# rchiaramo/wavefront_path_tracer

Hardware: AMD Instinct MI355X
Metric: Mrays/s (extend+shade) at 1920×1080, 64 spp, 8 bounces; 1/2/4/8 GPU (higher is better)
Workload: dtype f32

## Files before the change

include/wfpt.h:

```cpp
#ifndef WFPT_H
#define WFPT_H

#include <stddef.h>
#include <stdint.h>

#ifdef __cplusplus
extern "C" {
#endif


typedef struct wfpt_sphere {
    float center[4];
    float radius;
    uint32_t material_idx;
    uint32_t material_type;
    uint32_t _buffer;
} wfpt_sphere;

typedef struct wfpt_material {
    float albedo[4];
    float fuzz;
    float refract_index;
    uint32_t material_type;
    uint32_t _buffer;
// ... 69 lines not shown
                       offsetof(wfpt_ray, pixel_idx) == 44,
                   "Ray: extend.wgsl:17-22, 48 bytes");
WFPT_LAYOUT_ASSERT(sizeof(wfpt_hit_payload) == 16 && offsetof(wfpt_hit_payload, ray_idx) == 4 && offsetof(wfpt_hit_payload, sphere_idx) == 8 &&
                       offsetof(wfpt_hit_payload, mat_type) == 12,
                   "HitPayload: extend.wgsl:24-29, 16 bytes");


typedef enum wfpt_status {
    WFPT_OK = 0,
    WFPT_ERR_INVALID_ARGUMENT = -1,
    WFPT_ERR_HIP = -2,
    WFPT_ERR_OUT_OF_MEMORY = -3,
    WFPT_ERR_UNSUPPORTED = -4,
    WFPT_ERR_NO_DEVICE = -5
} wfpt_status;

typedef enum wfpt_stage {
    WFPT_STAGE_GENERATE_RAYS = 0,
    WFPT_STAGE_EXTEND = 1,
    WFPT_STAGE_SHADE = 2,
    WFPT_STAGE_MISS = 3,
    WFPT_STAGE_ACCUMULATE = 4,
    WFPT_STAGE_SHADE_LAMBERTIAN = 5,
    WFPT_STAGE_SHADE_METAL = 6,
    WFPT_STAGE_SHADE_DIELECTRIC = 7,
    WFPT_STAGE_SCAN = 8,
    WFPT_STAGE_BOUNCE_FIRST = 9,
    WFPT_STAGE_BOUNCE = 10,
    WFPT_STAGE_BOUNCE_LAST = 11,
    WFPT_STAGE_COMPACT = 12,
    WFPT_STAGE_COUNT = 13
} wfpt_stage;

typedef enum wfpt_rng_mode { WFPT_RNG_DISPATCH = 0, WFPT_RNG_PIXEL = 1 } wfpt_rng_mode;

enum {
    WFPT_FLAG_SPLIT_SHADE = 1u << 0,
    WFPT_FLAG_NO_GRAPH = 1u << 1,
    WFPT_FLAG_UNFUSED = 1u << 2,
    WFPT_FLAG_BINARY_BVH = 1u << 3,
    WFPT_FLAG_NO_REFILL = 1u << 4,
    WFPT_FLAG_NO_LDS_SCENE = 1u << 5,
    WFPT_FLAG_EXACT_TRAVERSAL = 1u << 6,
    WFPT_FLAG_NO_BINNING = 1u << 7,
    WFPT_FLAG_BINNING = 1u << 8,
    WFPT_FLAG_AOV = 1u << 10,
    WFPT_FLAG_DENOISE = 1u << 11,
    WFPT_FLAG_ENVIRONMENT = 1u << 12 ,
    WFPT_FLAG_TEXTURES = 1u << 13    ,
    WFPT_FLAG_EMISSION = 1u << 14    ,
    WFPT_FLAG_NEE = 1u << 15         ,
    WFPT_FLAG_ENV_NEE = 1u << 16     ,
    WFPT_FLAG_MIS = 1u << 17         ,
    WFPT_FLAG_ENV_MIS = 1u << 18
};

#define WFPT_INACTIVE_PIXEL 0xffffffffu

typedef struct wfpt_params {
    uint32_t width;
    uint32_t height;
    uint32_t max_pixels;
    uint32_t max_wavefronts;
    uint32_t miss_floor;
    uint32_t rng_mode;
    uint32_t flags;
    uint32_t tile_rank;
    uint32_t tile_world;
    int32_t device;
    uint32_t batch;
} wfpt_params;

typedef struct wfpt_ctx wfpt_ctx;


uint32_t wfpt_scene_new(wfpt_sphere *spheres, wfpt_material *materials);
uint32_t wfpt_scene_book_one_final(uint64_t seed, wfpt_sphere *spheres, wfpt_material *materials, uint32_t capacity);
int wfpt_build_bvh(wfpt_sphere *spheres, uint32_t n_spheres, wfpt_bvh_node *nodes, uint32_t node_capacity,
                   uint32_t *n_nodes);
int wfpt_build_bvh_triangles(wfpt_triangle *triangles, uint32_t n_triangles, wfpt_bvh_node *nodes,
                             uint32_t node_capacity, uint32_t *n_nodes, uint32_t n_bins);
int wfpt_build_bvh_device(wfpt_sphere *spheres, uint32_t n_spheres, wfpt_bvh_node *nodes, uint32_t node_capacity,
                          uint32_t *n_nodes, int device, float *device_ms);
int wfpt_build_bvh_triangles_device(wfpt_triangle *triangles, uint32_t n_triangles, wfpt_bvh_node *nodes,
                                    uint32_t node_capacity, uint32_t *n_nodes, uint32_t n_bins, int device,
                                    float *device_ms);
int wfpt_load_obj(const char *path, wfpt_triangle *triangles, uint32_t capacity, uint32_t *n_triangles,
                  uint32_t material_idx, uint32_t material_type);
int wfpt_load_obj_uv(const char *path, wfpt_triangle *triangles, float *uv6, uint32_t capacity, uint32_t *n_triangles,
                     uint32_t material_idx, uint32_t material_type);
uint32_t wfpt_scene_random_mesh(uint64_t seed, uint32_t n_triangles, wfpt_triangle *triangles, wfpt_material *materials);
void wfpt_camera_new(const float look_from[3], const float look_at[3], float *pitch, float *yaw);
void wfpt_view_transform(const float position[3], float pitch, float yaw, float view[16]);
void wfpt_p_inv(float vfov_rad, float aspect_ratio, float z_near, float z_far, float p_inv[16]);
void wfpt_gpu_camera_new(const float position[3], float pitch, float yaw, float defocus_angle_rad,
                         float focus_distance, wfpt_gpu_camera *out);
float wfpt_to_radians(float degrees);
void wfpt_camera_controller_update(float position[3], float *pitch, float *yaw, const float amounts[6],
                                   float rotate[2], float speed, float sensitivity, float dt);
void wfpt_workgroup_size_64(uint32_t x, uint32_t *gx, uint32_t *gy);
int wfpt_stage_from_name(const char *name);
const char *wfpt_stage_name(int stage);


int wfpt_device_count(void);
wfpt_ctx *wfpt_create(const wfpt_params *params,
                      const wfpt_sphere *spheres, uint32_t n_spheres,
// ... 146 lines not shown
int wfpt_emission_timing_ms(wfpt_ctx *ctx, float *ms_total, uint32_t *launches);

int wfpt_nee_light_count(wfpt_ctx *ctx);
int wfpt_nee_timing_ms(wfpt_ctx *ctx, float *ms_total, uint32_t *launches);
int wfpt_sample_lights(wfpt_ctx *ctx, const float *in9, size_t n, float *out8);

int wfpt_set_environment_share(wfpt_ctx *ctx, float share);
float wfpt_environment_share(const wfpt_ctx *ctx);
int wfpt_read_environment_distribution(wfpt_ctx *ctx, uint32_t *row_wh, uint64_t *marg_h);
int wfpt_sample_environment_light(wfpt_ctx *ctx, const float *in10, size_t n, float *out8);

int wfpt_sample_lights_mis(wfpt_ctx *ctx, const float *in9, size_t n, float *out12);
int wfpt_mis_hit_weight(wfpt_ctx *ctx, const float *in8, size_t n, float *out4);

int wfpt_sample_environment_light_mis(wfpt_ctx *ctx, const float *in10, size_t n, float *out12);
int wfpt_env_mis_miss_weight(wfpt_ctx *ctx, const float *dirs3, size_t n, float *out4);


uint32_t wfpt_n_pixels(const wfpt_ctx *ctx);
uint32_t wfpt_ray_capacity(const wfpt_ctx *ctx);
int wfpt_read_accumulated(wfpt_ctx *ctx, float *rgb, size_t n_floats);
int wfpt_read_image(wfpt_ctx *ctx, float *rgb, size_t n_floats);
int wfpt_copy_accumulated_to_device(wfpt_ctx *ctx, void *device_ptr, size_t n_bytes);
#define WFPT_COMM_UNIQUE_ID_BYTES 128
int wfpt_comm_unique_id(void *id128);
int wfpt_comm_init(wfpt_ctx *ctx, const void *id128, int rank, int world);
int wfpt_gather_accumulated(wfpt_ctx *ctx);
int wfpt_gather_accumulated_timed(wfpt_ctx *ctx, float *ms);
int wfpt_read_gathered(wfpt_ctx *ctx, float *rgb, size_t n_floats);
int wfpt_comm_destroy(wfpt_ctx *ctx);

int wfpt_read_rays(wfpt_ctx *ctx, wfpt_ray *rays, uint32_t n);
int wfpt_read_extension_rays(wfpt_ctx *ctx, wfpt_ray *rays, uint32_t n);
int wfpt_read_hits(wfpt_ctx *ctx, wfpt_hit_payload *hits, uint32_t n);
int wfpt_read_misses(wfpt_ctx *ctx, uint32_t *ray_indices, uint32_t n);
int wfpt_write_rays(wfpt_ctx *ctx, const wfpt_ray *rays, uint32_t n);
int wfpt_read_bounce_table(wfpt_ctx *ctx, uint32_t *rows4, uint32_t max_rows, uint32_t *n_rows);
int wfpt_read_totals(wfpt_ctx *ctx, uint64_t totals[3]);
int wfpt_read_wavefront_totals(wfpt_ctx *ctx, uint64_t *rows3, uint32_t max_rows, uint32_t *n_rows);
int wfpt_device_info(int device, uint32_t *compute_units, uint32_t *memory_clock_khz, uint32_t *memory_bus_width_bits,
                     uint64_t *total_memory_bytes);
void wfpt_tonemap_rgb8(const float *accumulated, uint32_t n_pixels, uint32_t n_samples, uint8_t *rgb);

int wfpt_save_ppm(wfpt_ctx *ctx, const char *path);
int wfpt_save_pfm(wfpt_ctx *ctx, const char *path);
int wfpt_save_png(wfpt_ctx *ctx, const char *path);
int wfpt_write_png_rgb8(const char *path, const uint8_t *rgb, uint32_t width, uint32_t height);

int wfpt_selftest_math(int device, int op, const float *a, const float *b, float *out, size_t n);
int wfpt_debug_extend_blocks_per_cu(int device, uint32_t lds_bytes);
int wfpt_debug_read_stamps(wfpt_ctx *ctx, uint64_t out[16], int reset);
int wfpt_debug_read_stamps_ex(wfpt_ctx *ctx, int which, uint64_t out[16], int reset);
int wfpt_debug_bvh4(const wfpt_bvh_node *nodes, uint32_t n_nodes, uint32_t counts[4]);
const char *wfpt_build_info(void);

#ifdef __cplusplus
}
#endif
#endif
```

wavefront_path_tracer_amd/__init__.py:

```python
import ctypes as C
import os

import numpy as np

from . import _build

__all__ = ["SPP", "SPF", "Scene", "BVHTree", "Camera", "CameraController", "ProjectionMatrix", "GPUFrameBuffer",
           "RenderParameters", "RenderProgress", "Kernel", "PathTracer", "WfptError", "workgroup_size_64",
           "RNG_DISPATCH", "RNG_PIXEL", "FLAG_SPLIT_SHADE", "FLAG_NO_GRAPH", "FLAG_UNFUSED", "FLAG_BINARY_BVH", "FLAG_NO_REFILL", "FLAG_NO_LDS_SCENE", "FLAG_EXACT_TRAVERSAL", "FLAG_NO_BINNING", "FLAG_BINNING", "FLAG_AOV", "AOVS", "FLAG_DENOISE", "DENOISE_DEFAULTS", "FLAG_ENVIRONMENT", "load_environment", "FLAG_TEXTURES", "MAX_TEXTURES", "load_texture", "FLAG_EMISSION", "FLAG_NEE", "FLAG_ENV_NEE", "FLAG_MIS", "FLAG_ENV_MIS", "TEMPORAL_DEFAULTS", "TEMPORAL_OUTPUTS", "STAGES", "lib", "build",
           "tonemap_rgb8", "selftest_math", "device_count"]

SPP = 10
SPF = 1

RNG_DISPATCH, RNG_PIXEL = 0, 1
LOOP_KINDS = ("stages", "fused", "fused_binned", "refill")
FLAG_SPLIT_SHADE, FLAG_NO_GRAPH, FLAG_UNFUSED, FLAG_BINARY_BVH, FLAG_NO_REFILL, FLAG_NO_LDS_SCENE, FLAG_EXACT_TRAVERSAL, FLAG_NO_BINNING, FLAG_BINNING = 1, 2, 4, 8, 16, 32, 64, 128, 256
FLAG_AOV = 1 << 10
FLAG_ENVIRONMENT = 1 << 12
FLAG_TEXTURES = 1 << 13
MAX_TEXTURES = 64
TEXTURE_FILTERS = {"bilinear": 0, "nearest": 1}
FLAG_EMISSION = 1 << 14
FLAG_NEE = 1 << 15
FLAG_ENV_NEE = 1 << 16
FLAG_MIS = 1 << 17
FLAG_ENV_MIS = 1 << 18
FLAG_DENOISE = 1 << 11
DENOISE_DEFAULTS = {"iterations": 5, "sigma_luminance": 4.0, "sigma_normal": 128.0, "sigma_depth": 1.0, "sigma_albedo": 0.5}
TEMPORAL_DEFAULTS = {**DENOISE_DEFAULTS, "history_cap": 32.0, "depth_tolerance": 0.05, "normal_cos": 0.9}
TEMPORAL_OUTPUTS = {"color": (0, 3), "moments": (1, 2), "length": (2, 1), "motion": (3, 3)}
INACTIVE_PIXEL = 0xFFFFFFFF
AOV_ALBEDO, AOV_NORMAL, AOV_DEPTH, AOV_COVERAGE, AOV_PRIM_ID, AOV_MATERIAL_ID = 0, 1, 2, 3, 4, 5
AOVS = {"albedo": (AOV_ALBEDO, 3, "<f4"), "normal": (AOV_NORMAL, 3, "<f4"), "depth": (AOV_DEPTH, 1, "<f4"),
        "coverage": (AOV_COVERAGE, 1, "<f4"), "prim_id": (AOV_PRIM_ID, 1, "<u4"), "material_id": (AOV_MATERIAL_ID, 1, "<u4")}
STAGES = {"generate_rays": 0, "extend": 1, "shade": 2, "miss_kernel": 3, "accumulate": 4,
          "shade_lambertian": 5, "shade_metal": 6, "shade_dielectric": 7, "scan": 8,
          "bounce_first": 9, "bounce": 10, "bounce_last": 11, "compact": 12}
STAGE_COUNT = 13

SPHERE = np.dtype([("center", "<f4", 4), ("radius", "<f4"), ("material_idx", "<u4"),
                   ("material_type", "<u4"), ("_buffer", "<u4")])
MATERIAL = np.dtype([("albedo", "<f4", 4), ("fuzz", "<f4"), ("refract_index", "<f4"),
                     ("material_type", "<u4"), ("_buffer", "<u4")])
BVH_NODE = np.dtype([("aabb_min", "<f4", 3), ("left_first", "<u4"), ("aabb_max", "<f4", 3),
                     ("prim_count", "<u4")])
GPU_CAMERA = np.dtype([("position", "<f4", 4), ("pitch", "<f4"), ("yaw", "<f4"),
                       ("defocus_radius", "<f4"), ("focus_distance", "<f4")])
RAY = np.dtype([("origin", "<f4", 4), ("direction", "<f4", 4), ("inv_direction", "<f4", 3),
                ("pixel_idx", "<u4")])
HIT = np.dtype([("t", "<f4"), ("ray_idx", "<u4"), ("sphere_idx", "<u4"), ("mat_type", "<u4")])
TRIANGLE = np.dtype([("v0", "<f4", 3), ("material_idx", "<u4"), ("e1", "<f4", 3), ("material_type", "<u4"),
                     ("e2", "<f4", 3), ("_pad", "<u4")])


OK, ERR_INVALID_ARGUMENT, ERR_HIP, ERR_OUT_OF_MEMORY, ERR_UNSUPPORTED, ERR_NO_DEVICE = 0, -1, -2, -3, -4, -5


class WfptError(RuntimeError):
    def __init__(self, status, message):
        super().__init__(f"wfpt status {status}: {message}")
        self.status = status


class _Params(C.Structure):
    _fields_ = [("width", C.c_uint32), ("height", C.c_uint32), ("max_pixels", C.c_uint32),
                ("max_wavefronts", C.c_uint32), ("miss_floor", C.c_uint32), ("rng_mode", C.c_uint32),
                ("flags", C.c_uint32), ("tile_rank", C.c_uint32), ("tile_world", C.c_uint32),
                ("device", C.c_int32), ("batch", C.c_uint32)]


class _DenoiseParams(C.Structure):
    _fields_ = [("iterations", C.c_uint32), ("sigma_luminance", C.c_float), ("sigma_normal", C.c_float), ("sigma_depth", C.c_float),
                ("sigma_albedo", C.c_float), ("_reserved", C.c_uint32 * 3)]


class _EnvironmentParams(C.Structure):
    _fields_ = [("intensity", C.c_float), ("rotation", C.c_float), ("_reserved", C.c_uint32 * 6)]


# ... 188 lines not shown
        "wfpt_build_info": (C.c_char_p, []),
        "wfpt_save_ppm": (i32, [vp, C.c_char_p]),
        "wfpt_save_pfm": (i32, [vp, C.c_char_p]),
        "wfpt_save_png": (i32, [vp, C.c_char_p]),
        "wfpt_write_png_rgb8": (i32, [C.c_char_p, vp, u32, u32]),
        "wfpt_debug_extend_blocks_per_cu": (i32, [i32, u32]),
        "wfpt_debug_read_stamps": (i32, [vp, vp, i32]),
        "wfpt_debug_read_stamps_ex": (i32, [vp, i32, vp, i32]),
        "wfpt_debug_bvh4": (i32, [vp, u32, vp]),
        "wfpt_aov_channels": (i32, [i32]),
        "wfpt_read_aov": (i32, [vp, i32, vp, sz]),
        "wfpt_copy_aov_to_device": (i32, [vp, i32, vp, sz]),
        "wfpt_aov_timing_ms": (i32, [vp, C.POINTER(f32), C.POINTER(u32)]),
        "wfpt_denoise_params_default": (None, [C.POINTER(_DenoiseParams)]),
        "wfpt_denoise": (i32, [vp, C.POINTER(_DenoiseParams), vp, sz]),
        "wfpt_denoise_to_device": (i32, [vp, C.POINTER(_DenoiseParams), vp, sz]),
        "wfpt_read_variance": (i32, [vp, vp, sz]),
        "wfpt_denoise_timing_ms": (i32, [vp, C.POINTER(f32), C.POINTER(u32)]),
        "wfpt_set_frame_offset": (i32, [vp, u32]),
        "wfpt_frame_offset": (u32, [vp]),
        "wfpt_temporal_params_default": (None, [C.POINTER(_TemporalParams)]),
        "wfpt_denoise_temporal": (i32, [vp, C.POINTER(_TemporalParams), vp, sz]),
        "wfpt_denoise_temporal_to_device": (i32, [vp, C.POINTER(_TemporalParams), vp, sz]),
        "wfpt_read_temporal": (i32, [vp, i32, vp, sz]),
        "wfpt_reset_history": (i32, [vp]),
        "wfpt_temporal_timing_ms": (i32, [vp, C.POINTER(f32), C.POINTER(u32)]),
        "wfpt_environment_params_default": (None, [C.POINTER(_EnvironmentParams)]),
        "wfpt_set_environment": (i32, [vp, vp, u32, u32, C.POINTER(_EnvironmentParams)]),
        "wfpt_clear_environment": (i32, [vp]),
        "wfpt_sample_environment": (i32, [vp, vp, sz, vp]),
        "wfpt_texture_params_default": (None, [C.POINTER(_TextureParams)]),
        "wfpt_set_texture": (i32, [vp, u32, vp, u32, u32, C.POINTER(_TextureParams)]),
        "wfpt_clear_texture": (i32, [vp, u32]),
        "wfpt_bind_texture": (i32, [vp, u32, C.c_int32]),
        "wfpt_set_triangle_uvs": (i32, [vp, vp, u32]),
        "wfpt_sample_texture": (i32, [vp, u32, vp, sz, vp]),
        "wfpt_texture_timing_ms": (i32, [vp, C.POINTER(f32), C.POINTER(u32)]),
        "wfpt_load_obj_uv": (i32, [C.c_char_p, vp, vp, u32, C.POINTER(u32), u32, u32]),
        "wfpt_set_emission": (i32, [vp, u32, C.POINTER(f32)]),
        "wfpt_get_emission": (i32, [vp, u32, C.POINTER(f32)]),
        "wfpt_clear_emission": (i32, [vp]),
        "wfpt_emission_timing_ms": (i32, [vp, C.POINTER(f32), C.POINTER(u32)]),
        "wfpt_nee_light_count": (i32, [vp]),
        "wfpt_nee_timing_ms": (i32, [vp, C.POINTER(f32), C.POINTER(u32)]),
        "wfpt_sample_lights": (i32, [vp, vp, sz, vp]),
        "wfpt_set_environment_share": (i32, [vp, f32]),
        "wfpt_environment_share": (f32, [vp]),
        "wfpt_read_environment_distribution": (i32, [vp, vp, vp]),
        "wfpt_sample_environment_light": (i32, [vp, vp, sz, vp]),
        "wfpt_sample_lights_mis": (i32, [vp, vp, sz, vp]),
        "wfpt_mis_hit_weight": (i32, [vp, vp, sz, vp]),
        "wfpt_sample_environment_light_mis": (i32, [vp, vp, sz, vp]),
        "wfpt_env_mis_miss_weight": (i32, [vp, vp, sz, vp]),
    }
    for name, (res, args) in sig.items():
        fn = getattr(L, name)
        fn.restype = res
        fn.argtypes = args
    _lib = L
    return L


ABI_SYMBOLS = None


def abi_symbols():
    import re
    hdr = os.path.join(_build.ROOT, "include", "wfpt.h")
    text = open(hdr).read()
    text = re.sub(r"/\*.*?\*/", "", text, flags=re.S)
    return sorted(set(re.findall(r"\b(wfpt_[a-z0-9_]+)\s*\(", text)))


def _p(a):
    return a.ctypes.data_as(C.c_void_p)


def device_count():
    return lib().wfpt_device_count()


def comm_unique_id():
    buf = np.zeros(128, np.uint8)
    st = lib().wfpt_comm_unique_id(_p(buf))
    if st != 0:
        raise WfptError(st, lib().wfpt_last_error(None).decode())
    return buf.tobytes()


def device_info(device=0):
    cu, clk, width, mem = C.c_uint32(), C.c_uint32(), C.c_uint32(), C.c_uint64()
    st = lib().wfpt_device_info(device, C.byref(cu), C.byref(clk), C.byref(width), C.byref(mem))
    if st != 0:
        raise WfptError(st, lib().wfpt_last_error(None).decode())
    return {"compute_units": cu.value, "memory_clock_khz": clk.value, "memory_bus_width_bits": width.value,
            "total_memory_bytes": mem.value}


def workgroup_size_64(x):
    gx, gy = C.c_uint32(), C.c_uint32()
    lib().wfpt_workgroup_size_64(x, C.byref(gx), C.byref(gy))
    return gx.value, gy.value


def tonemap_rgb8(accumulated, n_samples):
    a = np.ascontiguousarray(accumulated, "<f4").reshape(-1)
    out = np.zeros(a.size, np.uint8)
    lib().wfpt_tonemap_rgb8(_p(a), a.size // 3, n_samples, _p(out))
    return out.reshape(-1, 3)


def write_png(path, rgb8, width, height):
    a = np.ascontiguousarray(rgb8, np.uint8)
    if a.size != 3 * width * height:
        raise ValueError("rgb8 must hold width * height RGB pixels")
    st = lib().wfpt_write_png_rgb8(os.fsencode(path), _p(a), width, height)
    if st != 0:
        raise WfptError(st, f"cannot write {path}")


def load_environment(path):
    data = open(path, "rb").read()
    if data[:2] in (b"PF", b"Pf"):
        return _read_pfm(data)
    if data[:2] == b"#?":
        return _read_hdr(data)
    raise ValueError(f"load_environment: {path} is neither a Radiance .hdr nor a .pfm file")

# ... 665 lines not shown
        n = int(np.prod(shape))
        want = ("float32",) if dtype == "<f4" else ("int32", "uint32")
        dt = str(getattr(tensor, "dtype", "")).replace("torch.", "")
        if dt not in want:
            raise TypeError(f"aov_to_tensor({name!r}): tensor dtype {dt or type(tensor).__name__} is not {' or '.join(want)}")
        if tensor.numel() != n:
            raise ValueError(f"aov_to_tensor({name!r}): tensor has {tensor.numel()} elements, the AOV {n} {shape}")
        if not tensor.is_contiguous():
            raise ValueError(f"aov_to_tensor({name!r}): tensor is not contiguous")
        if getattr(tensor, "device", None) is None or tensor.device.type != "cuda" or tensor.device.index != self._params.device:
            raise ValueError(f"aov_to_tensor({name!r}): tensor must live on this context's device (cuda:{self._params.device})")
        self._check(lib().wfpt_copy_aov_to_device(self.handle, which, C.c_void_p(tensor.data_ptr()), 4 * n))
        return tensor

    def aov_timing(self):
        ms, n = C.c_float(0.0), C.c_uint32(0)
        self._check(lib().wfpt_aov_timing_ms(self.handle, C.byref(ms), C.byref(n)))
        return float(ms.value), int(n.value)

    def variance(self):
        a = np.zeros((self.n_pixels // self.width, self.width), "<f4")
        self._check(lib().wfpt_read_variance(self.handle, _p(a), a.size))
        return a

    @staticmethod
    def _denoise_params(params):
        unknown = set(params) - set(DENOISE_DEFAULTS)
        if unknown:
            raise TypeError(f"unknown denoise parameter(s) {sorted(unknown)}: one of {sorted(DENOISE_DEFAULTS)}")
        v = {**DENOISE_DEFAULTS, **params}
        return _DenoiseParams(int(v["iterations"]), v["sigma_luminance"], v["sigma_normal"], v["sigma_depth"], v["sigma_albedo"])

    def denoise(self, **params):
        p = self._denoise_params(params)
        a = np.zeros((self.n_pixels // self.width, self.width, 3), "<f4")
        self._check(lib().wfpt_denoise(self.handle, C.byref(p), _p(a), a.size))
        return a

    def denoise_to_tensor(self, tensor, **params):
        p = self._denoise_params(params)
        n = self.n_pixels * 3
        dt = str(getattr(tensor, "dtype", "")).replace("torch.", "")
        if dt != "float32":
            raise TypeError(f"denoise_to_tensor: tensor dtype {dt or type(tensor).__name__} is not float32")
        if tensor.numel() != n:
            raise ValueError(f"denoise_to_tensor: tensor has {tensor.numel()} elements, the image {n}")
        if not tensor.is_contiguous():
            raise ValueError("denoise_to_tensor: tensor is not contiguous")
        if getattr(tensor, "device", None) is None or tensor.device.type != "cuda" or tensor.device.index != self._params.device:
            raise ValueError(f"denoise_to_tensor: tensor must live on this context's device (cuda:{self._params.device})")
        self._check(lib().wfpt_denoise_to_device(self.handle, C.byref(p), C.c_void_p(tensor.data_ptr()), 4 * n))
        return tensor

    def denoise_timing(self):
        ms, n = C.c_float(0.0), C.c_uint32(0)
        self._check(lib().wfpt_denoise_timing_ms(self.handle, C.byref(ms), C.byref(n)))
        return float(ms.value), int(n.value)

    def set_frame_offset(self, offset):
        self._check(lib().wfpt_set_frame_offset(self.handle, int(offset) & 0xFFFFFFFF))

    @property
    def frame_offset(self):
        return int(lib().wfpt_frame_offset(self.handle))

    @staticmethod
    def _temporal_params(params):
        unknown = set(params) - set(TEMPORAL_DEFAULTS)
        if unknown:
            raise TypeError(f"unknown temporal denoise parameter(s) {sorted(unknown)}: one of {sorted(TEMPORAL_DEFAULTS)}")
        v = {**TEMPORAL_DEFAULTS, **params}
        spatial = PathTracer._denoise_params({k: v[k] for k in DENOISE_DEFAULTS})
        return _TemporalParams(spatial, v["history_cap"], v["depth_tolerance"], v["normal_cos"])

    def denoise_temporal(self, **params):
        p = self._temporal_params(params)
        a = np.zeros((self.n_pixels // self.width, self.width, 3), "<f4")
        self._check(lib().wfpt_denoise_temporal(self.handle, C.byref(p), _p(a), a.size))
        return a

    def denoise_temporal_to_tensor(self, tensor, **params):
        p = self._temporal_params(params)
        n = self.n_pixels * 3
        dt = str(getattr(tensor, "dtype", "")).replace("torch.", "")
        if dt != "float32":
            raise TypeError(f"denoise_temporal_to_tensor: tensor dtype {dt or type(tensor).__name__} is not float32")
        if tensor.numel() != n:
            raise ValueError(f"denoise_temporal_to_tensor: tensor has {tensor.numel()} elements, the image {n}")
        if not tensor.is_contiguous():
            raise ValueError("denoise_temporal_to_tensor: tensor is not contiguous")
        if getattr(tensor, "device", None) is None or tensor.device.type != "cuda" or tensor.device.index != self._params.device:
            raise ValueError(f"denoise_temporal_to_tensor: tensor must live on this context's device (cuda:{self._params.device})")
        self._check(lib().wfpt_denoise_temporal_to_device(self.handle, C.byref(p), C.c_void_p(tensor.data_ptr()), 4 * n))
        return tensor

    def temporal(self, name):
        if name not in TEMPORAL_OUTPUTS:
            raise KeyError(f"unknown temporal output {name!r}: one of {sorted(TEMPORAL_OUTPUTS)}")
        which, ch = TEMPORAL_OUTPUTS[name]
        h = self.n_pixels // self.width
        a = np.zeros((h, self.width, ch) if ch > 1 else (h, self.width), "<f4")
        self._check(lib().wfpt_read_temporal(self.handle, which, _p(a), a.size))
        return a

    def reset_history(self):
        self._check(lib().wfpt_reset_history(self.handle))
# ... 270 lines not shown
```

wavefront_path_tracer_amd/_build.py:

```python
import os
import shutil
import subprocess

PKG_DIR = os.path.dirname(os.path.abspath(__file__))
ROOT = os.path.dirname(PKG_DIR)
CSRC = os.path.join(PKG_DIR, "csrc")
LIB_PATH = os.path.join(PKG_DIR, "libwfpt.so")
SOURCES = ["wfpt_kernels.hip", "wfpt_api.hip", "wfpt_bvh_build.hip", "wfpt_host.cpp"]
HEADERS = [os.path.join(CSRC, "wfpt_kernels.h"), os.path.join(CSRC, "wfpt_bvh4.h"), os.path.join(CSRC, "wfpt_device_math.h"),
           os.path.join(ROOT, "include", "wfpt.h")]
FLAGS = ["--offload-arch=gfx950", "-O3", "-std=c++17", "-fPIC", "-shared", "-ffp-contract=off",
         "-fhip-fp32-correctly-rounded-divide-sqrt", "-fno-fast-math", "-Wall", "-Wno-unused-function"]


def hipcc():
    exe = shutil.which("hipcc") or "/opt/rocm/bin/hipcc"
    if not os.path.exists(exe):
        raise RuntimeError("hipcc not found: libwfpt.so cannot be built (and there is no CPU fallback)")
    return exe


def stale():
    if not os.path.exists(LIB_PATH):
        return True
    t = os.path.getmtime(LIB_PATH)
    deps = [os.path.join(CSRC, s) for s in SOURCES] + HEADERS + [os.path.abspath(__file__)]
    return any(os.path.getmtime(d) > t for d in deps)


BUILD_INFO = os.path.join(PKG_DIR, "build_info.json")


def source_digest():
    import hashlib
    h = hashlib.sha256()
    for f in [os.path.join(CSRC, s) for s in SOURCES] + HEADERS:
        h.update(os.path.basename(f).encode() + b"\0")
        h.update(open(f, "rb").read())
    return h.hexdigest()


def write_build_info():
    import datetime
    import json

    def git(*a):
        try:
            return subprocess.run(["git", "-C", ROOT] + list(a), stdout=subprocess.PIPE, stderr=subprocess.DEVNULL, text=True, timeout=20).stdout.strip()
        except Exception:
            return ""
    info = {"git_head": git("rev-parse", "HEAD") or None, "git_dirty": bool(git("status", "--porcelain", "--untracked-files=no")),
            "built_utc": datetime.datetime.utcnow().strftime("%Y-%m-%dT%H:%M:%SZ"), "source_sha256": source_digest(),
            "flags": FLAGS + os.environ.get("WFPT_EXTRA_FLAGS", "").split()}
    try:
        json.dump(info, open(BUILD_INFO, "w"), indent=1)
    except OSError:
        pass
    return info


def build_info():
    import json
# ... 33 lines not shown
```

wavefront_path_tracer_amd/csrc/wfpt_api.hip:

```cpp
#include "wfpt_kernels.h"

#include <dlfcn.h>
#include <rccl/rccl.h>

#include <algorithm>
#include <cfloat>
#include <cmath>
#include <cstdio>
#include <cstdlib>
#include <cstring>
#include <deque>
#include <map>
#include <memory>
#include <string>
#include <type_traits>
#include <vector>

using namespace wfpt;

namespace {
thread_local std::string g_last_error;
thread_local int g_last_status = 0;

template <auto Free> struct HipDeleter {
// ... 166 lines not shown
        uint32_t width = 0, height = 0;
    } tp[2];
    HistoryBuffers tp_buf;
    int tp_live = 0;
    bool tp_read_ok = false;
    uint64_t epoch = 0;
    EventPair tp_ev;
    float tp_ms = 0.0f;
    uint32_t tp_calls = 0;
    DeviceBuffer<float4> env_tex;
    EnvDev env{};
    DeviceBuffer<float4> tex_texels[WFPT_MAX_TEXTURES];
    TexDev tex_dev[WFPT_MAX_TEXTURES] = {};
    std::vector<int32_t> tex_bind;
    DeviceBuffer<float> tex_uv;
    uint32_t tex_uv_rows = 0;
    DeviceBuffer<TexDev> tex_desc;
    DeviceBuffer<uint2> tex_prim;
    std::vector<uint32_t> h_prim_mat_idx, h_prim_row;
    double tex_ms = 0.0;
    uint32_t tex_launches = 0;
    std::vector<float> em_rgb;
    DeviceBuffer<uint32_t> em_prim;
    DeviceBuffer<float4> em_mat;
    DeviceBuffer<float> emitted;
    double em_ms = 0.0;
    uint32_t em_launches = 0;
    DeviceBuffer<uint32_t> nee_lights;
    uint32_t n_lights = 0;
    uint32_t stage_extends = 0;
    double nee_ms = 0.0;
    uint32_t nee_launches = 0;
    DeviceBuffer<float4> mis_origin;
    DeviceBuffer<uint32_t> env_row;
    DeviceBuffer<uint64_t> env_marg;
    uint64_t env_total = 0;
    float env_share = 0.5f;
    uint32_t frame_offset = 0;
    DeviceBuffer<Control> ctl;
    DeviceBuffer<CameraDev> camera;
    wfpt_gpu_camera h_camera{};
    float h_inv_proj[16] = {}, h_view[16] = {};
    SceneBuffers sb;
    SceneDev scene{};
    float extent[3] = {0, 0, 0};
    bool ch_ok = false;
    bool far_rays = false;
    uint32_t depth4 = 0;
    std::vector<uint32_t> h_prim_mat_type;

    uint32_t accumulate_grid = 0;
    uint32_t progress_frame = 0, accumulated_samples = 0;
    bool dev_frame_valid = false;

    std::map<uint32_t, Graph> graphs;

    StageTimer timers[WFPT_STAGE_COUNT];
    std::vector<EventPair> sample_events;
    std::string err;
};

namespace {

int fail(wfpt_ctx *c, int code, const std::string &msg) {
    if (c) c->err = msg;
    g_last_error = msg;
    g_last_status = code;
    return code;
}
int hip_fail(wfpt_ctx *c, hipError_t e, const char *what) {
    return fail(c, e == hipErrorOutOfMemory ? WFPT_ERR_OUT_OF_MEMORY : WFPT_ERR_HIP,
                std::string(what) + ": " + hipGetErrorString(e));
}
#define WFPT_HIP(c, call)                                   \
    do {                                                    \
        hipError_t e_ = (call);                             \
        if (e_ != hipSuccess) return hip_fail(c, e_, #call); \
    } while (0)

void set_queue(RayQueue &q, float *base, size_t cap) {
    q.base = base;
    q.cap = static_cast<uint32_t>(cap);
}

struct Viewport {
    uint32_t tiles_x, tiles_y_local;
    uint64_t n_pixels;
};
Viewport viewport_of(uint32_t w, uint32_t h, Tiling tile) {
    const uint32_t tiles_y = h / 8u + (h % 8u != 0u);
    const uint32_t tiles_y_local = tiles_y > tile.rank ? (tiles_y - tile.rank + tile.world - 1) / tile.world : 0;
    return Viewport{w / 8u + (w % 8u != 0u), tiles_y_local,
                    tile.world <= 1 ? static_cast<uint64_t>(w) * h : static_cast<uint64_t>(tiles_y_local) * 8u * w};
}
void set_viewport(wfpt_ctx *c, uint32_t w, uint32_t h) {
    const Viewport v = viewport_of(w, h, c->tile);
    c->width = w;
    c->height = h;
    c->tiles_x = v.tiles_x;
    c->tiles_y_local = v.tiles_y_local;
    c->n_pixels = static_cast<uint32_t>(v.n_pixels);
    c->has_inactive = (w % 8u) != 0 || (h % 8u) != 0;
}

int validate_bvh(wfpt_ctx *c, const wfpt_bvh_node *nodes, uint32_t n_nodes, uint32_t n_spheres,
                 std::vector<uint32_t> &pair_parent) {
// ... 286 lines not shown
    a.sample_out = out;
    a.sample_n = static_cast<uint32_t>(n);
    return a;
}
hipError_t launch_connect_pass(wfpt_ctx *c, const ConnectArgs &a, uint32_t nb) {
    return launch_connect(a, extend_grid(c, nb), c->stream.get(), textured(c), env_connecting(c), weighing(c) || env_weighing(c));
}
hipError_t launch_emission_pass(wfpt_ctx *c, const EmissionArgs &a, uint32_t grid) {
    return launch_emission(a, !connecting(c) ? kEmitAll : env_weighing(c) ? kEmitWeighedEnv : weighing(c) ? kEmitWeighed : kEmitGated, grid,
                           c->stream.get(), 1.0f - env_dist(c).share);
}
const float *miss_gate(const wfpt_ctx *c) { return env_connecting(c) ? c->emitted.get() : nullptr; }
constexpr int kStageConnect = WFPT_STAGE_COUNT + 3;

ScanBinnedArgs scan_binned_args(wfpt_ctx *c, uint32_t bounce, uint32_t nb, int parity) {
    ScanBinnedArgs a{};
    a.batch = batch_of(c, nb);
    a.chunk_hits = c->f_chunk_hits[parity].get();
    a.chunk_miss = c->f_chunk_miss[parity].get();
    a.chunk_cls = c->f_cls[parity].get();
    a.cls_table = c->cls_table.get();
    a.first_seg_cls = c->first_seg_cls.get();
    a.ctl = c->ctl.get();
    a.n_in = &c->ctl.get()->n_in;
    a.limit = c->capacity;
    a.miss_floor = c->p.miss_floor;
    a.bounce = bounce;
    return a;
}
PlanArgs plan_args(wfpt_ctx *c, uint32_t nb, bool last) {
    PlanArgs a{};
    a.batch = batch_of(c, nb);
    a.ctl = c->ctl.get();
    a.plan = c->plan.get();
    a.plan_seg_off = nb * kBinClasses + 1u;
    a.plan_miss_off = a.plan_seg_off + nb + 1u;
    a.last = last ? 1u : 0u;
    return a;
}
const EnvDev *env_of(const wfpt_ctx *c) { return c->env_tex.get() ? &c->env : nullptr; }
hipError_t launch_miss_pass(wfpt_ctx *c, const MissArgs &a, uint32_t grid) {
    const EnvDist d = env_dist(c);
    return launch_miss(a, grid, c->stream.get(), env_of(c) ? &d : nullptr, miss_gate(c), env_weighing(c));
}
bool use_binned(const wfpt_ctx *c) {
    return c->bin_capable && !c->env_tex.get() && !textured(c) && !emitting(c) && c->fused && c->scene.lds_scene && !c->rec_dense.get() && c->scene.n_spheres <= (1u << 16) &&
           c->batch_max * static_cast<uint32_t>(kBinClasses) <= 1024u && c->p.rng_mode == WFPT_RNG_PIXEL;
}
wfpt_loop_kind loop_of(const wfpt_ctx *c) {
    if (!c->fused) return WFPT_LOOP_STAGES;
    if (c->rec_dense.get() && !c->scene.exact) return WFPT_LOOP_REFILL;
    return use_binned(c) ? WFPT_LOOP_FUSED_BINNED : WFPT_LOOP_FUSED;
}
uint32_t bounce_grid(const wfpt_ctx *c, uint32_t n) {
    const uint64_t items = (static_cast<uint64_t>(c->n_chunks_max) * 5u / 4u + 1u) * n;
    return static_cast<uint32_t>(std::min<uint64_t>(items, static_cast<uint64_t>(c->cus) * c->bounce_blocks_per_cu));
}

struct EventRec { int stage; hipEvent_t start, stop; };


template <typename Timed>
int enqueue_pre_shade(wfpt_ctx *c, Timed &timed, uint32_t b, uint32_t nb, const HitWalk &w) {
    const uint32_t grid = consumer_grid(c, nb);
    if (textured(c)) WFPT_HIP(c, timed(kStageTexture, [&] { return launch_texture(texture_args(c, w), grid, c->stream.get()); }));
    if (emitting(c)) WFPT_HIP(c, timed(kStageEmission, [&] { return launch_emission_pass(c, emission_args(c, w), grid); }));
    if (connecting(c)) WFPT_HIP(c, timed(kStageConnect, [&] { return launch_connect_pass(c, connect_args(c, b, w), nb); }));
    return WFPT_OK;
}

template <typename Timed>
int enqueue_stages(wfpt_ctx *c, Timed &timed, uint32_t nb) {
    const hipStream_t st = c->stream.get();
    const bool split = (c->p.flags & WFPT_FLAG_SPLIT_SHADE) != 0;
    const EnvDev *env = env_of(c);
    WFPT_HIP(c, timed(WFPT_STAGE_GENERATE_RAYS, [&] { return launch_generate(generate_args(c, c->tiles_x, c->tiles_y_local, true, nb), st); }));
    for (uint32_t b = 0; b < c->p.max_wavefronts; ++b) {
        const int qi = static_cast<int>(b & 1u);
        WFPT_HIP(c, timed(WFPT_STAGE_EXTEND, [&] {
                     return launch_extend(extend_args(c, qi, &c->ctl.get()->n_in, c->capacity, nb, split), extend_grid(c, nb), st, env != nullptr);
                 }));
        WFPT_HIP(c, timed(WFPT_STAGE_SCAN, [&] { return launch_scan(scan_args(c, &c->ctl.get()->n_in, c->capacity, true, b, nb), st); }));
        const HitWalk w = hit_walk(c, -1, nb, qi, &c->ctl.get()->shade_n, c->capacity);
        if (int r = enqueue_pre_shade(c, timed, b, nb, w); r != WFPT_OK) return r;
        WFPT_HIP(c, timed(split ? WFPT_STAGE_SHADE_LAMBERTIAN : WFPT_STAGE_SHADE, [&] {
                     ShadeArgs sa = shade_args(c, qi, &c->ctl.get()->shade_n, c->capacity, 0, 0xffffffffu, false, nb);
                     sa.rec_in = c->hit_rec.get();
                     return launch_shade(sa, consumer_grid(c, nb), st);
                 }));
        WFPT_HIP(c, timed(WFPT_STAGE_MISS, [&] {
                     return launch_miss_pass(c, miss_args(c, qi, &c->ctl.get()->miss_n, c->capacity, nb), consumer_grid(c, nb));
                 }));
    }
    return WFPT_OK;
}

template <typename Timed>
int enqueue_fused(wfpt_ctx *c, Timed &timed, uint32_t nb) {
    const hipStream_t st = c->stream.get();
    const uint32_t grid = bounce_grid(c, nb);
    const EnvDev *env = env_of(c);
    WFPT_HIP(c, timed(WFPT_STAGE_BOUNCE_FIRST, [&] { return launch_bounce(bounce_args(c, 1, 0, nb), kBounceFirst, grid, st, env != nullptr); }));
    for (uint32_t b = 0; b < c->p.max_wavefronts; ++b) {
        const int par = static_cast<int>(b & 1u);
        const bool last = b + 1 >= c->p.max_wavefronts;
        WFPT_HIP(c, timed(WFPT_STAGE_SCAN, [&] { return launch_scan(scan_args(c, &c->ctl.get()->n_in, c->capacity, true, b, nb, par), st); }));
        if (env) WFPT_HIP(c, timed(WFPT_STAGE_MISS, [&] { return launch_miss_pass(c, fused_miss_args(c, par, nb), consumer_grid(c, nb)); }));
        if (int r = enqueue_pre_shade(c, timed, b, nb, hit_walk(c, par, nb)); r != WFPT_OK) return r;
        WFPT_HIP(c, timed(last ? WFPT_STAGE_BOUNCE_LAST : WFPT_STAGE_BOUNCE, [&] {
                     return launch_bounce(bounce_args(c, par, par ^ 1, nb), last ? kBounceLast : kBounceMiddle, grid, st, env != nullptr);
                 }));
    }
    return WFPT_OK;
}

template <typename Timed>
int enqueue_fused_binned(wfpt_ctx *c, Timed &timed, uint32_t nb) {
    const hipStream_t st = c->stream.get();
    const uint64_t items = (static_cast<uint64_t>(c->n_chunks_max) * 5u / 4u + 1u) * nb;
    const uint32_t grid = static_cast<uint32_t>(std::min<uint64_t>(items, static_cast<uint64_t>(c->cus) * c->bounce_binned_blocks_per_cu));
    WFPT_HIP(c, timed(WFPT_STAGE_BOUNCE_FIRST, [&] { return launch_bounce_binned(bounce_args(c, 1, 0, nb), kBounceFirst, grid, st); }));
    for (uint32_t b = 0; b < c->p.max_wavefronts; ++b) {
        const int par = static_cast<int>(b & 1u);
        const bool last = b + 1 >= c->p.max_wavefronts;
        WFPT_HIP(c, timed(WFPT_STAGE_SCAN, [&] {
                     hipError_t e = launch_scan_binned(scan_binned_args(c, b, nb, par), st);
                     return e != hipSuccess ? e : launch_plan(plan_args(c, nb, last), st);
                 }));
        WFPT_HIP(c, timed(last ? WFPT_STAGE_BOUNCE_LAST : WFPT_STAGE_BOUNCE,
                          [&] { return launch_bounce_binned(bounce_args(c, par, par ^ 1, nb), last ? kBounceLast : kBounceMiddle, grid, st); }));
    }
    return WFPT_OK;
}

template <typename Timed>
int enqueue_refill(wfpt_ctx *c, Timed &timed, uint32_t nb) {
    const hipStream_t st = c->stream.get();
    const uint32_t grid = c->cus * c->bounce_blocks_per_cu;
    const EnvDev *env = env_of(c);
    WFPT_HIP(c, timed(WFPT_STAGE_GENERATE_RAYS, [&] { return launch_generate_dense(refill_args(c, 1, nb), st); }));
    WFPT_HIP(c, timed(WFPT_STAGE_BOUNCE_FIRST, [&] { return launch_refill(refill_args(c, 1, nb), kBounceFirst, grid, st); }));
    for (uint32_t b = 0; b < c->p.max_wavefronts; ++b) {
        const int par = static_cast<int>(b & 1u);
        WFPT_HIP(c, timed(WFPT_STAGE_COMPACT, [&] { return launch_compact(compact_args(c, par, nb), c->n_chunks_max, st, env != nullptr); }));
        WFPT_HIP(c, timed(WFPT_STAGE_SCAN, [&] { return launch_scan(scan_args(c, &c->ctl.get()->n_in, c->capacity, true, b, nb, par), st); }));
        const bool last = b + 1 >= c->p.max_wavefronts;
        if (!last || env)
            WFPT_HIP(c, timed(WFPT_STAGE_MISS, [&] { return launch_miss_pass(c, fused_miss_args(c, par, nb), consumer_grid(c, nb)); }));
        if (int r = enqueue_pre_shade(c, timed, b, nb, hit_walk(c, par, nb)); r != WFPT_OK) return r;
        if (!last) {
            WFPT_HIP(c, timed(WFPT_STAGE_SHADE, [&] { return launch_shade_rays(refill_args(c, par, nb), c->n_chunks_max, st); }));
            WFPT_HIP(c, timed(WFPT_STAGE_BOUNCE, [&] { return launch_refill(refill_args(c, par, nb), kBounceMiddle, grid, st); }));
        } else {
            WFPT_HIP(c, timed(WFPT_STAGE_BOUNCE_LAST,
                              [&] { return launch_bounce(bounce_args(c, par, par ^ 1, nb), kBounceLast, bounce_grid(c, nb), st, env != nullptr); }));
// ... 27 lines not shown
        return launch_accumulate_emission(a, c->emitted.get(), c->moments.get(), c->pixel_capacity, c->accumulate_grid, c->stream.get());
    if (c->moments.get()) return launch_accumulate_moments(a, c->moments.get(), c->pixel_capacity, c->accumulate_grid, c->stream.get());
    return launch_accumulate(a, c->accumulate_grid, c->stream.get());
}

int enqueue_batch(wfpt_ctx *c, std::vector<EventRec> *ev, uint32_t nb) {
    size_t next_event = 0;
    auto timed = [&](int stage, auto &&launch) -> hipError_t {
        if (!ev) return launch();
        if (next_event == c->sample_events.size()) c->sample_events.emplace_back();
        EventPair &p = c->sample_events[next_event++];
        hipError_t r = p.create();
        if (r == hipSuccess) r = hipEventRecord(p.start.get(), c->stream.get());
        if (r == hipSuccess) r = launch();
        if (r != hipSuccess) return r;
        ev->push_back({stage, p.start.get(), p.stop.get()});
        return hipEventRecord(p.stop.get(), c->stream.get());
    };
    c->cur = 0;
    if (c->aov_sums.get())
        WFPT_HIP(c, timed(kStageAov, [&] {
                     const TexScene ts = tex_scene(c);
                     return launch_aov(aov_args(c, nb), aov_grid(c), c->stream.get(), env_of(c), textured(c) ? &ts : nullptr);
                 }));
    if (second_plane(c))
        WFPT_HIP(c, timed(kStageEmission, [&] {
                     return hipMemsetAsync(c->emitted.get(), 0, sizeof(float) * nb * c->image_floats, c->stream.get());
                 }));
    int r = WFPT_OK;
    switch (loop_of(c)) {
    case WFPT_LOOP_STAGES: r = enqueue_stages(c, timed, nb); break;
    case WFPT_LOOP_FUSED: r = enqueue_fused(c, timed, nb); break;
    case WFPT_LOOP_FUSED_BINNED: r = enqueue_fused_binned(c, timed, nb); break;
    case WFPT_LOOP_REFILL: r = enqueue_refill(c, timed, nb); break;
    }
    if (r != WFPT_OK) return r;
    WFPT_HIP(c, timed(WFPT_STAGE_ACCUMULATE, [&] { return launch_batch_accumulate(c, nb); }));
    return WFPT_OK;
}

int clear_sums(wfpt_ctx *c) {
    WFPT_HIP(c, hipMemsetAsync(c->accumulated.get(), 0, sizeof(float) * c->acc_floats, c->stream.get()));
    c->epoch += 1;
    if (c->aov_sums.get()) WFPT_HIP(c, hipMemsetAsync(c->aov_sums.get(), 0, sizeof(float) * c->aov_sums.size(), c->stream.get()));
    if (c->moments.get()) WFPT_HIP(c, hipMemsetAsync(c->moments.get(), 0, sizeof(float) * c->moments.size(), c->stream.get()));
    return WFPT_OK;
}

void drop_history(wfpt_ctx *c) {
    c->tp[0].valid = c->tp[1].valid = false;
    c->tp_read_ok = false;
}

int scene_changed(wfpt_ctx *c) {
    c->graphs.clear();
    c->hit_rec_valid = false;
    drop_history(c);
    return wfpt_reset_progress(c);
}

void batch_rendered(wfpt_ctx *c, uint32_t nb) {
    c->cur = static_cast<int>(c->p.max_wavefronts & 1u);
    c->hit_rec_valid = false;
    c->progress_frame += nb;
    c->accumulated_samples += nb;
    c->last_slot = nb - 1;
}

int ensure_device_frame(wfpt_ctx *c) {
    if (c->dev_frame_valid) return WFPT_OK;
    const wfpt_frame_buffer f{c->width, c->height, c->progress_frame + 1u + c->frame_offset, 0u};
    WFPT_HIP(c, launch_set_frame(c->ctl.get(), f, c->stream.get()));
    c->dev_frame_valid = true;
    return WFPT_OK;
}

int render_batch(wfpt_ctx *c, uint32_t nb) {
    WFPT_HIP(c, hipSetDevice(c->device));
    if (int r = ensure_device_frame(c); r != WFPT_OK) return r;
    if (c->p.flags & WFPT_FLAG_NO_GRAPH) {
        if (int r = enqueue_batch(c, nullptr, nb); r != WFPT_OK) return r;
    } else {
        auto it = c->graphs.find(nb);
        if (it == c->graphs.end()) {
            hipGraph_t g = nullptr;
            hipGraphExec_t ge = nullptr;
            WFPT_HIP(c, hipStreamBeginCapture(c->stream.get(), hipStreamCaptureModeThreadLocal));
            const int r = enqueue_batch(c, nullptr, nb);
            const hipError_t e = hipStreamEndCapture(c->stream.get(), &g);
            Graph owned;
            owned.graph.reset(g);
            if (r != WFPT_OK) return r;
            if (e != hipSuccess) return hip_fail(c, e, "hipStreamEndCapture");
            if (const hipError_t ie = hipGraphInstantiate(&ge, g, nullptr, nullptr, 0); ie != hipSuccess) return hip_fail(c, ie, "hipGraphInstantiate");
            owned.exec.reset(ge);
            it = c->graphs.emplace(nb, std::move(owned)).first;
        }
        WFPT_HIP(c, hipGraphLaunch(it->second.exec.get(), c->stream.get()));
    }
    batch_rendered(c, nb);
    return WFPT_OK;
}

int render_many(wfpt_ctx *c, uint32_t n_samples) {
    while (n_samples > 0) {
        const uint32_t nb = std::min(n_samples, c->batch_max);
        if (int r = render_batch(c, nb); r != WFPT_OK) return r;
        n_samples -= nb;
    }
    return WFPT_OK;
}

int stage_begin(wfpt_ctx *c, int stage) {
    StageTimer &t = c->timers[stage];
    WFPT_HIP(c, t.ev.create());
    WFPT_HIP(c, hipEventRecord(t.ev.start.get(), c->stream.get()));
    return WFPT_OK;
}
int stage_end(wfpt_ctx *c, int stage) {
    StageTimer &t = c->timers[stage];
    WFPT_HIP(c, hipEventRecord(t.ev.stop.get(), c->stream.get()));
    t.pending = true;
    return WFPT_OK;
}

constexpr int kMarginLog2 = -17;

bool scene_extent(const wfpt_bvh_node *nodes, uint32_t n_nodes, const float cam_reach[3], float extent[3]) {
    for (int ax = 0; ax < 3; ++ax) {
        float e = 0.25f * cam_reach[ax];
        for (uint32_t i = 0; i < n_nodes; ++i) {
            if (i == 1) continue;
// ... 449 lines not shown
                              params->rng_mode == WFPT_RNG_PIXEL && (params->flags & WFPT_FLAG_BINNING) != 0;
    if (want_binning && cap + kBinClasses * kChunk <= 0xffffffffull) {
        cap += kBinClasses * kChunk;
        c->bin_capable = true;
    }
    c->capacity = static_cast<uint32_t>(cap);
    c->n_chunks_max = c->capacity / kChunk;
    c->fused = (params->flags & (WFPT_FLAG_UNFUSED | WFPT_FLAG_SPLIT_SHADE)) == 0 && c->n_chunks_max <= 65535u;
    c->bin_capable = c->bin_capable && c->fused;
    c->batch_max = params->batch == 0 ? 16u : std::min<uint32_t>(params->batch, c->fused ? kMaxBatch : kMaxBatchClassic);
    c->classic_batch = c->fused ? 1u : c->batch_max;
    const size_t nb_all = c->batch_max;
    const size_t nb = c->classic_batch;
    if (7ull * cap > 0xffffffffull || 4ull * c->pixel_capacity > 0xffffffffull) {
        fail(nullptr, WFPT_ERR_UNSUPPORTED, "wfpt_create: ray capacity beyond 2^32 / 7 slots (or 2^30 pixels): slice strides are 32-bit");
        wfpt_destroy(c);
        return nullptr;
    }
    if (nb * c->capacity > 0xffffffffull || nb_all * c->capacity > 0xffffffffull) {
        fail(nullptr, WFPT_ERR_UNSUPPORTED, "wfpt_create: samples in flight x ray capacity beyond 2^32 queue slots");
        wfpt_destroy(c);
        return nullptr;
    }

    for (int k = 0; k < 2; ++k) {
        CREATE_HIP(c->ray_mem[k].alloc_zeroed(nb * 7 * static_cast<size_t>(c->capacity), st));
        set_queue(c->q[k], c->ray_mem[k].get(), c->capacity);
    }
    CREATE_HIP(c->hit_mem.alloc(3 * nb * c->capacity));
    CREATE_HIP(c->hit_rec.alloc(2 * nb * c->capacity));
    const size_t miss_planes = (params->flags & WFPT_FLAG_ENVIRONMENT) ? kMissPlanesEnv : kMissPlanes;
    CREATE_HIP(c->miss_mem.alloc(miss_planes * nb * c->capacity));
    c->hq.base = c->hit_mem.get(); c->hq.plane = nb * c->capacity;
    c->mq.base = c->miss_mem.get(); c->mq.plane = nb * c->capacity;
    const size_t n_counts = nb_all * c->n_chunks_max;
    for (auto *b : {&c->chunk_hits, &c->chunk_miss, &c->chunk_hit_base, &c->chunk_miss_base}) CREATE_HIP(b->alloc_zeroed(n_counts, st));
    CREATE_HIP(c->mat_list.alloc(3 * nb * c->capacity));
    CREATE_HIP(c->chunk_mat.alloc_zeroed(3 * n_counts, st));
    c->image_floats = 4 * static_cast<size_t>(c->pixel_capacity);
    c->acc_floats = (3 * static_cast<size_t>(c->pixel_capacity) + 7) / 4 * 4;
    CREATE_HIP(c->image.alloc(nb_all * c->image_floats));
    CREATE_HIP(launch_fill(c->image.get(), 1.0f, nb_all * c->image_floats, st));
    CREATE_HIP(c->accumulated.alloc_zeroed(c->acc_floats, st));
    if (c->fused) {
        const size_t slots = nb_all * c->capacity, counts = nb_all * c->n_chunks_max;
        for (int k = 0; k < 2; ++k) {
            CREATE_HIP(c->rec_mem[k].alloc(2 * slots));
            CREATE_HIP(c->f_miss_mem[k].alloc(miss_planes * slots));
            c->f_mq[k].base = c->f_miss_mem[k].get(); c->f_mq[k].plane = slots;
            CREATE_HIP(c->f_chunk_hits[k].alloc_zeroed(counts, st));
            CREATE_HIP(c->f_chunk_miss[k].alloc_zeroed(counts, st));
        }
        CREATE_HIP(c->first_seg.alloc_zeroed(counts, st));
        if (c->bin_capable) {
            for (int k = 0; k < 2; ++k) CREATE_HIP(c->f_cls[k].alloc_zeroed(counts * ClsPack<kBinClasses>::kWords, st));
            CREATE_HIP(c->cls_table.alloc_zeroed(counts * kBinClasses, st));
            CREATE_HIP(c->first_seg_cls.alloc_zeroed(counts * kBinClasses, st));
            CREATE_HIP(c->plan.alloc_zeroed(kPlanWords, st));
        }
    }
    if (c->p.flags & WFPT_FLAG_AOV) CREATE_HIP(c->aov_sums.alloc_zeroed(kAovPlanes * static_cast<size_t>(c->pixel_capacity), st));
    if (c->p.flags & WFPT_FLAG_DENOISE) CREATE_HIP(c->moments.alloc_zeroed(kMomentPlanes * static_cast<size_t>(c->pixel_capacity), st));
    CREATE_HIP(c->ctl.alloc_zeroed(kMaxBatch, st));
    CREATE_HIP(c->camera.alloc(1));
    CREATE_HIP(c->d_stamps.alloc_zeroed(48, st));

    hipDeviceProp_t prop;
    CREATE_HIP(hipGetDeviceProperties(&prop, c->device));
    c->cus = static_cast<uint32_t>(prop.multiProcessorCount);
    const uint32_t cus = c->cus;
    c->h_camera = *camera;
    std::memcpy(c->h_inv_proj, inv_proj, sizeof c->h_inv_proj);
    std::memcpy(c->h_view, view, sizeof c->h_view);
    if (upload_scene(c, spheres, triangles, n_spheres, materials, n_materials, nodes, n_nodes, pair_parent, static_cast<uint32_t>(bvh_depth),
                     camera) != WFPT_OK) {
        g_last_error = c->err;
        wfpt_destroy(c);
        return nullptr;
    }

    CameraDev cam{};
    cam.cam = *camera;
    std::memcpy(cam.inv_proj, inv_proj, sizeof cam.inv_proj);
    std::memcpy(cam.view, view, sizeof cam.view);
    CREATE_HIP(hipMemcpy(c->camera.get(), &cam, sizeof cam, hipMemcpyHostToDevice));
    const wfpt_frame_buffer f{c->width, c->height, 0u, 0u};
    CREATE_HIP(hipMemcpy(&c->ctl.get()->frame, &f, sizeof f, hipMemcpyHostToDevice));

    c->accumulate_grid = std::min<uint32_t>((c->pixel_capacity + 255u) / 256u, cus * 32u);
    if (c->accumulate_grid == 0) c->accumulate_grid = 1;
    CREATE_HIP(hipStreamSynchronize(st));
#undef CREATE_HIP
    return c;
}

wfpt_ctx *wfpt_create(const wfpt_params *params, const wfpt_sphere *spheres, uint32_t n_spheres,
                      const wfpt_material *materials, uint32_t n_materials, const wfpt_bvh_node *nodes,
                      uint32_t n_nodes, const wfpt_gpu_camera *camera, const float inv_proj[16], const float view[16]) {
    if (!spheres) {
        fail(nullptr, WFPT_ERR_INVALID_ARGUMENT, "wfpt_create: null or empty argument");
        return nullptr;
    }
    return create_impl(params, spheres, nullptr, n_spheres, materials, n_materials, nodes, n_nodes, camera, inv_proj, view);
}

wfpt_ctx *wfpt_create_mesh(const wfpt_params *params, const wfpt_triangle *triangles, uint32_t n_triangles,
                           const wfpt_material *materials, uint32_t n_materials, const wfpt_bvh_node *nodes,
                           uint32_t n_nodes, const wfpt_gpu_camera *camera, const float inv_proj[16], const float view[16]) {
    if (!triangles) {
        fail(nullptr, WFPT_ERR_INVALID_ARGUMENT, "wfpt_create_mesh: null or empty argument");
        return nullptr;
    }
    return create_impl(params, nullptr, triangles, n_triangles, materials, n_materials, nodes, n_nodes, camera, inv_proj, view);
}

static int render_chunked_impl(const wfpt_params *params, const wfpt_sphere *spheres, const wfpt_triangle *triangles, uint32_t n_prims,
                               const wfpt_material *materials, uint32_t n_materials, const wfpt_bvh_node *nodes, uint32_t n_nodes,
                               const wfpt_gpu_camera *camera, const float inv_proj[16], const float view[16], uint32_t n_samples,
                               uint32_t chunks, float *rgb) {
    if (!params || !rgb || chunks == 0) return fail(nullptr, WFPT_ERR_INVALID_ARGUMENT, "wfpt_render_chunked: null or empty argument");
    if (chunks > 1 && params->rng_mode != WFPT_RNG_PIXEL)
        return fail(nullptr, WFPT_ERR_INVALID_ARGUMENT,
                    "wfpt_render_chunked: WFPT_RNG_DISPATCH keys shade's RNG on a ray's queue position, which depends on the cut; "
                    "use WFPT_RNG_PIXEL to get the unchunked image");
    const uint32_t w = params->width, h = params->height;
    const size_t band_floats = 8u * static_cast<size_t>(w) * 3u;
    std::vector<float> slab;
    for (uint32_t k = 0; k < chunks; ++k) {
        wfpt_params p = *params;
        p.tile_rank = k;
        p.tile_world = chunks;
        p.max_pixels = 0;
        p.flags &= ~static_cast<uint32_t>(WFPT_FLAG_AOV | WFPT_FLAG_DENOISE | WFPT_FLAG_ENVIRONMENT | WFPT_FLAG_TEXTURES | WFPT_FLAG_EMISSION | WFPT_FLAG_NEE | WFPT_FLAG_ENV_NEE | WFPT_FLAG_MIS | WFPT_FLAG_ENV_MIS);
        if (bands_of(h, k, chunks) == 0) continue;
        g_last_status = WFPT_ERR_HIP;
        wfpt_ctx *c = create_impl(&p, spheres, triangles, n_prims, materials, n_materials, nodes, n_nodes, camera, inv_proj, view);
        if (!c) return g_last_status;
        int r = wfpt_render(c, n_samples);
        if (r == WFPT_OK) {
            slab.resize(3 * static_cast<size_t>(c->n_pixels));
            r = wfpt_read_accumulated(c, slab.data(), slab.size());
        }
        if (r != WFPT_OK) {
            g_last_error = c->err;
            wfpt_destroy(c);
            return r;
        }
        const uint32_t nb = bands_of(h, k, chunks);
        for (uint32_t j = 0; j < nb; ++j) {
            const uint32_t y0 = (j * chunks + k) * 8u, rows = std::min(8u, h - y0);
            std::memcpy(rgb + static_cast<size_t>(y0) * w * 3u, slab.data() + j * band_floats, sizeof(float) * rows * w * 3u);
        }
        wfpt_destroy(c);
    }
    return WFPT_OK;
}

int wfpt_render_chunked(const wfpt_params *params, const wfpt_sphere *spheres, uint32_t n_spheres, const wfpt_material *materials,
                        uint32_t n_materials, const wfpt_bvh_node *nodes, uint32_t n_nodes, const wfpt_gpu_camera *camera,
                        const float inv_proj[16], const float view[16], uint32_t n_samples, uint32_t chunks, float *rgb) {
    if (!spheres) return fail(nullptr, WFPT_ERR_INVALID_ARGUMENT, "wfpt_render_chunked: null argument");
    return render_chunked_impl(params, spheres, nullptr, n_spheres, materials, n_materials, nodes, n_nodes, camera, inv_proj, view, n_samples, chunks, rgb);
}

int wfpt_render_chunked_mesh(const wfpt_params *params, const wfpt_triangle *triangles, uint32_t n_triangles, const wfpt_material *materials,
                             uint32_t n_materials, const wfpt_bvh_node *nodes, uint32_t n_nodes, const wfpt_gpu_camera *camera,
                             const float inv_proj[16], const float view[16], uint32_t n_samples, uint32_t chunks, float *rgb) {
    if (!triangles) return fail(nullptr, WFPT_ERR_INVALID_ARGUMENT, "wfpt_render_chunked_mesh: null argument");
    return render_chunked_impl(params, nullptr, triangles, n_triangles, materials, n_materials, nodes, n_nodes, camera, inv_proj, view, n_samples, chunks, rgb);
}

void wfpt_destroy(wfpt_ctx *c) {
    if (!c) return;
    (void)hipSetDevice(c->device);
    if (c->stream.get()) (void)hipStreamSynchronize(c->stream.get());
    (void)wfpt_comm_destroy(c);
    delete c;
}

int wfpt_set_frame(wfpt_ctx *c, const wfpt_frame_buffer *frame) {
    if (!c || !frame) return fail(c, WFPT_ERR_INVALID_ARGUMENT, "wfpt_set_frame: null argument");
    WFPT_HIP(c, hipSetDevice(c->device));
    WFPT_HIP(c, hipMemcpyAsync(&c->ctl.get()->frame, frame, sizeof *frame, hipMemcpyHostToDevice, c->stream.get()));
    WFPT_HIP(c, hipStreamSynchronize(c->stream.get()));
    c->dev_frame_valid = false;
    return WFPT_OK;
}

int wfpt_update_render_parameters(wfpt_ctx *c, uint32_t width, uint32_t height, const wfpt_gpu_camera *camera,
                                  const float inv_proj[16], const float view[16]) {
    if (!c || !camera || !inv_proj || !view || width == 0 || height == 0)
        return fail(c, WFPT_ERR_INVALID_ARGUMENT, "wfpt_update_render_parameters: null or empty argument");
    if (static_cast<uint64_t>(width) * height > (1ull << 31))
        return fail(c, WFPT_ERR_INVALID_ARGUMENT, "wfpt_update_render_parameters: image too large");
    const Viewport v = viewport_of(width, height, c->tile);
    const uint64_t slots = static_cast<uint64_t>(v.tiles_x) * v.tiles_y_local * 64u;
    if (v.n_pixels > c->pixel_capacity || slots > c->capacity)
        return fail(c, WFPT_ERR_INVALID_ARGUMENT, "viewport exceeds the capacity given at wfpt_create (max_pixels)");
    WFPT_HIP(c, hipSetDevice(c->device));
    c->hit_rec_valid = false;
    WFPT_HIP(c, hipStreamSynchronize(c->stream.get()));
    if (width != c->width || height != c->height) drop_history(c);
    set_viewport(c, width, height);
    CameraDev cam{};
    cam.cam = *camera;
    std::memcpy(cam.inv_proj, inv_proj, sizeof cam.inv_proj);
    std::memcpy(cam.view, view, sizeof cam.view);
    WFPT_HIP(c, hipMemcpy(c->camera.get(), &cam, sizeof cam, hipMemcpyHostToDevice));
    if (int r = wfpt_reset_progress(c); r != WFPT_OK) return r;
    c->graphs.clear();
    c->h_camera = *camera;
    std::memcpy(c->h_inv_proj, inv_proj, sizeof c->h_inv_proj);
    std::memcpy(c->h_view, view, sizeof c->h_view);
    float reach[3];
    camera_reach(*camera, reach);
    c->scene.exact = decide_exact(c->p.flags, c->scene, c->ch_ok, c->extent, c->far_rays, reach);
    return alloc_gather_buffers(c);
}

static int build_texture_tables(wfpt_ctx *c, const TexDev *dev, const std::vector<int32_t> &bind, const std::vector<uint32_t> &mat_idx,
                                const std::vector<uint32_t> &row, TextureTables &out);
static void commit_texture_tables(wfpt_ctx *c, TextureTables &&t);
static int build_emission_tables(wfpt_ctx *c, const std::vector<float> &rgb, const std::vector<uint32_t> &mat_idx, EmissionTables &out);
static void commit_emission_tables(wfpt_ctx *c, EmissionTables &&t);
static int update_scene_impl(wfpt_ctx *c, wfpt_sphere *spheres, wfpt_triangle *triangles, uint32_t n_prims, const wfpt_material *materials,
                             uint32_t n_materials, uint32_t n_bins) {
    if (!c || !(spheres || triangles) || !materials || n_prims == 0 || n_materials == 0)
        return fail(c, WFPT_ERR_INVALID_ARGUMENT, "wfpt_update_scene: null or empty argument");
    for (uint32_t i = 0; i < n_prims; ++i)
        if ((spheres ? spheres[i].material_idx : triangles[i].material_idx) >= n_materials)
            return fail(c, WFPT_ERR_INVALID_ARGUMENT, "wfpt_update_scene: primitive material_idx out of range");
    if (triangles && (c->p.flags & WFPT_FLAG_TEXTURES) && c->tex_uv_rows)
        for (uint32_t i = 0; i < n_prims; ++i)
            if (triangles[i]._pad >= c->tex_uv_rows)
                return fail(c, WFPT_ERR_INVALID_ARGUMENT, "wfpt_update_scene_mesh: a triangle's UV row (_pad) is beyond the UV table");
    WFPT_HIP(c, hipSetDevice(c->device));
    WFPT_HIP(c, hipStreamSynchronize(c->stream.get()));
    std::vector<wfpt_bvh_node> nodes(2 * static_cast<size_t>(n_prims));
    uint32_t n_nodes = 0;
    const int st = spheres ? wfpt_build_bvh_device(spheres, n_prims, nodes.data(), static_cast<uint32_t>(nodes.size()), &n_nodes, c->device, nullptr)
                           : wfpt_build_bvh_triangles_device(triangles, n_prims, nodes.data(), static_cast<uint32_t>(nodes.size()), &n_nodes,
                                                             n_bins ? n_bins : 32u, c->device, nullptr);
    if (st != WFPT_OK) return fail(c, st, std::string("wfpt_update_scene: BVH build failed: ") + g_last_error);
    std::vector<uint32_t> pair_parent;
    const int depth = validate_bvh(c, nodes.data(), n_nodes, n_prims, pair_parent);
    if (depth < 0) return depth;
    TextureTables tables;
    if (c->p.flags & WFPT_FLAG_TEXTURES) {
        std::vector<uint32_t> mat_idx(n_prims), row(n_prims);
        for (uint32_t i = 0; i < n_prims; ++i) {
            mat_idx[i] = spheres ? spheres[i].material_idx : triangles[i].material_idx;
            row[i] = spheres ? 0u : triangles[i]._pad;
        }
        if (int r = build_texture_tables(c, c->tex_dev, c->tex_bind, mat_idx, row, tables); r != WFPT_OK) return r;
    }
    EmissionTables em_tables;
    std::vector<float> em_rgb;
    if (c->p.flags & WFPT_FLAG_EMISSION) {
        em_rgb = c->em_rgb;
        em_rgb.resize(3 * static_cast<size_t>(n_materials), 0.0f);
        std::vector<uint32_t> mat_idx(n_prims);
        for (uint32_t i = 0; i < n_prims; ++i) mat_idx[i] = spheres ? spheres[i].material_idx : triangles[i].material_idx;
        if (int r = build_emission_tables(c, em_rgb, mat_idx, em_tables); r != WFPT_OK) return r;
// ... 119 lines not shown
        WFPT_HIP(c, launch_shade(shade_args(c, c->cur, n_hits, threads, gx, material, true), consumer_grid(c, 1), c->stream.get()));
        break;
    }
    case WFPT_STAGE_MISS:
        WFPT_HIP(c, launch_miss_pass(c, miss_args(c, c->cur, &c->ctl.get()->counters[0], threads), consumer_grid(c, 1)));
        break;
    case WFPT_STAGE_ACCUMULATE:
        if (second_plane(c))
            WFPT_HIP(c, launch_accumulate_emission(accumulate_args(c, threads, false), c->emitted.get(), nullptr, 0, c->accumulate_grid, c->stream.get()));
        else
            WFPT_HIP(c, launch_accumulate(accumulate_args(c, threads, false), c->accumulate_grid, c->stream.get()));
        break;
    default: break;
    }
    return stage_end(c, stage);
}

float wfpt_kernel_timing_us(wfpt_ctx *c, int stage) {
    if (!c || stage < 0 || stage >= WFPT_STAGE_COUNT) return 0.0f;
    StageTimer &t = c->timers[stage];
    if (t.pending) {
        (void)hipSetDevice(c->device);
        if (hipEventSynchronize(t.ev.stop.get()) == hipSuccess) {
            float ms = 0.0f;
            if (hipEventElapsedTime(&ms, t.ev.start.get(), t.ev.stop.get()) == hipSuccess) {
                if (t.window.size() == 10) t.window.pop_back();
                t.window.push_front(static_cast<double>(ms) * 1000.0);
            }
        }
        t.pending = false;
    }
    if (t.window.empty()) return 0.0f;
    double sum = 0.0;
    for (double v : t.window) sum += v;
    return static_cast<float>(sum / static_cast<double>(t.window.size()));
}

int wfpt_render_sample(wfpt_ctx *c) {
    if (!c) return fail(c, WFPT_ERR_INVALID_ARGUMENT, "null context");
    return render_batch(c, 1);
}

int wfpt_render(wfpt_ctx *c, uint32_t n_samples) {
    if (!c) return fail(c, WFPT_ERR_INVALID_ARGUMENT, "null context");
    return render_many(c, n_samples);
}

int wfpt_render_timed(wfpt_ctx *c, uint32_t n_samples, float *stage_ms, uint32_t *stage_launches) {
    if (!c || !stage_ms) return fail(c, WFPT_ERR_INVALID_ARGUMENT, "wfpt_render_timed: null argument");
    WFPT_HIP(c, hipSetDevice(c->device));
    while (n_samples > 0) {
        const uint32_t nb = std::min(n_samples, c->batch_max);
        if (int r = ensure_device_frame(c); r != WFPT_OK) return r;
        std::vector<EventRec> ev;
        if (int r = enqueue_batch(c, &ev, nb); r != WFPT_OK) return r;
        WFPT_HIP(c, hipStreamSynchronize(c->stream.get()));
        for (const EventRec &e : ev) {
            float ms = 0.0f;
            WFPT_HIP(c, hipEventElapsedTime(&ms, e.start, e.stop));
            if (e.stage == kStageAov) {
                c->aov_ms += ms;
                c->aov_launches += 1;
                continue;
            }
            if (e.stage == kStageTexture) {
                c->tex_ms += ms;
                c->tex_launches += 1;
                continue;
            }
            if (e.stage == kStageEmission) {
                c->em_ms += ms;
                c->em_launches += 1;
                continue;
            }
            if (e.stage == kStageConnect) {
                c->nee_ms += ms;
                c->nee_launches += 1;
                continue;
            }
            stage_ms[e.stage] += ms;
            if (stage_launches) stage_launches[e.stage] += 1;
        }
        batch_rendered(c, nb);
        n_samples -= nb;
    }
    return WFPT_OK;
}

int wfpt_render_sample_timed(wfpt_ctx *c, float *stage_ms, uint32_t *stage_launches) {
    if (!c) return fail(c, WFPT_ERR_INVALID_ARGUMENT, "null context");
    const uint32_t keep = c->batch_max;
    c->batch_max = 1;
    const int r = wfpt_render_timed(c, 1, stage_ms, stage_launches);
    c->batch_max = keep;
    return r;
}

int wfpt_synchronize(wfpt_ctx *c) {
    if (!c) return fail(c, WFPT_ERR_INVALID_ARGUMENT, "null context");
    WFPT_HIP(c, hipSetDevice(c->device));
    WFPT_HIP(c, hipStreamSynchronize(c->stream.get()));
    return WFPT_OK;
}

uint32_t wfpt_frame(const wfpt_ctx *c) { return c ? c->progress_frame : 0; }
int wfpt_set_frame_offset(wfpt_ctx *c, uint32_t offset) {
// ... 672 lines not shown
    FILE *f = std::fopen(path, "wb");
    if (!f) return fail(c, WFPT_ERR_INVALID_ARGUMENT, std::string("wfpt_save_ppm: cannot open ") + path);
    std::fprintf(f, "P6\n%u %u\n255\n", c->width, c->height);
    const bool ok = std::fwrite(rgb.data(), 1, rgb.size(), f) == rgb.size();
    std::fclose(f);
    return ok ? WFPT_OK : fail(c, WFPT_ERR_INVALID_ARGUMENT, "wfpt_save_ppm: short write");
}

int wfpt_save_png(wfpt_ctx *c, const char *path) {
    std::vector<float> acc;
    if (int r = read_frame(c, acc, "wfpt_save_png"); r != WFPT_OK) return r;
    if (!path) return fail(c, WFPT_ERR_INVALID_ARGUMENT, "wfpt_save_png: null path");
    std::vector<uint8_t> rgb(acc.size());
    wfpt_tonemap_rgb8(acc.data(), c->n_pixels, c->accumulated_samples, rgb.data());
    const int st = wfpt_write_png_rgb8(path, rgb.data(), c->width, c->height);
    return st == WFPT_OK ? WFPT_OK : fail(c, st, std::string("wfpt_save_png: cannot write ") + path);
}

int wfpt_save_pfm(wfpt_ctx *c, const char *path) {
    std::vector<float> acc;
    if (int r = read_frame(c, acc, "wfpt_save_pfm"); r != WFPT_OK) return r;
    if (!path) return fail(c, WFPT_ERR_INVALID_ARGUMENT, "wfpt_save_pfm: null path");
    const float inv_n = 1.0f / static_cast<float>(c->accumulated_samples);
    for (float &v : acc) v = inv_n * v;
    FILE *f = std::fopen(path, "wb");
    if (!f) return fail(c, WFPT_ERR_INVALID_ARGUMENT, std::string("wfpt_save_pfm: cannot open ") + path);
    std::fprintf(f, "PF\n%u %u\n-1.0\n", c->width, c->height);
    bool ok = true;
    const size_t row = 3 * static_cast<size_t>(c->width);
    for (uint32_t y = c->height; y-- > 0 && ok;) ok = std::fwrite(acc.data() + y * row, sizeof(float), row, f) == row;
    std::fclose(f);
    return ok ? WFPT_OK : fail(c, WFPT_ERR_INVALID_ARGUMENT, "wfpt_save_pfm: short write");
}

int wfpt_debug_read_stamps(wfpt_ctx *c, uint64_t out[16], int reset) {
    if (!c || !out) return fail(c, WFPT_ERR_INVALID_ARGUMENT, "wfpt_debug_read_stamps: null argument");
    WFPT_HIP(c, hipSetDevice(c->device));
    WFPT_HIP(c, hipStreamSynchronize(c->stream.get()));
    WFPT_HIP(c, hipMemcpy(out, c->d_stamps.get(), sizeof(uint64_t) * 16, hipMemcpyDeviceToHost));
    if (reset) WFPT_HIP(c, hipMemset(c->d_stamps.get(), 0, sizeof(uint64_t) * 16));
    return WFPT_OK;
}

int wfpt_debug_read_stamps_ex(wfpt_ctx *c, int which, uint64_t out[16], int reset) {
    if (which == 0) return wfpt_debug_read_stamps(c, out, reset);
    if (!c || !out || which < 0 || which > 2) return fail(c, WFPT_ERR_INVALID_ARGUMENT, "wfpt_debug_read_stamps_ex: bad argument");
    WFPT_HIP(c, hipSetDevice(c->device));
    WFPT_HIP(c, hipStreamSynchronize(c->stream.get()));
    WFPT_HIP(c, hipMemcpy(out, c->d_stamps.get() + 16 * which, sizeof(uint64_t) * 16, hipMemcpyDeviceToHost));
    if (reset) WFPT_HIP(c, hipMemset(c->d_stamps.get() + 16 * which, 0, sizeof(uint64_t) * 16));
    return WFPT_OK;
}

int wfpt_debug_extend_blocks_per_cu(int device, uint32_t lds_bytes) {
    int n_dev = 0;
    if (hipGetDeviceCount(&n_dev) != hipSuccess || device < 0 || device >= n_dev)
        return fail(nullptr, WFPT_ERR_NO_DEVICE, "wfpt_debug_extend_blocks_per_cu: no HIP device");
    WFPT_HIP(nullptr, hipSetDevice(device));
    SceneDev sc{};
    sc.lds_scene = 1;
    sc.lds_bytes = lds_bytes;
    int blocks = 0;
    WFPT_HIP(nullptr, extend_blocks_per_cu(sc, &blocks));
    return blocks;
}

void wfpt_environment_params_default(wfpt_environment_params *p) {
    if (!p) return;
    *p = wfpt_environment_params{};
    p->intensity = 1.0f;
    p->rotation = 0.0f;
}

static int environment_check(wfpt_ctx *c, const char *who) {
    if (!c) return fail(c, WFPT_ERR_INVALID_ARGUMENT, std::string(who) + ": null context");
    if (!(c->p.flags & WFPT_FLAG_ENVIRONMENT))
        return fail(c, WFPT_ERR_INVALID_ARGUMENT, std::string(who) + ": the context was created without WFPT_FLAG_ENVIRONMENT");
    if (wfpt_loop_kind_of(c) == WFPT_LOOP_FUSED_BINNED)
        return fail(c, WFPT_ERR_UNSUPPORTED, std::string(who) + ": the class-binned loop (WFPT_FLAG_BINNING) takes no environment map");
    return WFPT_OK;
}

struct EnvTables {
    DeviceBuffer<uint32_t> row;
    DeviceBuffer<uint64_t> marg;
    uint64_t total = 0;
    DeviceBuffer<float> plane;
    DeviceBuffer<float4> origin;
};
static int build_env_tables(wfpt_ctx *c, const EnvDev &env, EnvTables &out) {
    if (!(c->p.flags & WFPT_FLAG_ENV_NEE)) return WFPT_OK;
    const size_t n = static_cast<size_t>(env.w) * env.h;
    const hipStream_t st = c->stream.get();
    DeviceBuffer<float> f;
    DeviceBuffer<uint32_t> max_bits;
    WFPT_HIP(c, f.alloc(n));
    WFPT_HIP(c, max_bits.alloc(1));
    WFPT_HIP(c, hipMemsetAsync(max_bits.get(), 0, sizeof(uint32_t), st));
    WFPT_HIP(c, launch_env_weights(env, f.get(), max_bits.get(), st));
    float M = 0.0f;
    WFPT_HIP(c, hipMemcpyAsync(&M, max_bits.get(), sizeof(float), hipMemcpyDeviceToHost, st));
    WFPT_HIP(c, hipStreamSynchronize(st));
    if (!(M > 0.0f && M <= FLT_MAX)) return WFPT_OK;
    WFPT_HIP(c, out.row.alloc(n));
    WFPT_HIP(c, out.marg.alloc(env.h));
    WFPT_HIP(c, launch_env_tables(env, f.get(), M, out.row.get(), out.marg.get(), st));
// ... 559 lines not shown
```

wavefront_path_tracer_amd/csrc/wfpt_host.cpp:

```cpp
#include "wfpt.h"
#include "wfpt_bvh4.h"

#include <algorithm>
#include <cmath>
#include <cstdio>
#include <cstdlib>
#include <cstring>
#include <utility>
#include <limits>
#include <vector>

namespace {

struct Vec3 {
    float x, y, z;
    float operator[](int i) const { return i == 0 ? x : (i == 1 ? y : z); }
};
inline Vec3 operator-(Vec3 a, Vec3 b) { return {a.x - b.x, a.y - b.y, a.z - b.z}; }
inline float zmin(float a, float b) { return a != a ? b : (b != b ? a : (a < b ? a : (b < a ? b : (std::signbit(a) ? a : b)))); }
inline float zmax(float a, float b) { return a != a ? b : (b != b ? a : (a > b ? a : (b > a ? b : (std::signbit(a) ? b : a)))); }
inline Vec3 vmin(Vec3 a, Vec3 b) { return {zmin(a.x, b.x), zmin(a.y, b.y), zmin(a.z, b.z)}; }
inline Vec3 vmax(Vec3 a, Vec3 b) { return {zmax(a.x, b.x), zmax(a.y, b.y), zmax(a.z, b.z)}; }
inline float dot(Vec3 a, Vec3 b) { return (a.x * b.x + a.y * b.y) + a.z * b.z; }
inline float length(Vec3 a) { return std::sqrt(dot(a, a)); }
inline Vec3 cross(Vec3 a, Vec3 b) {
    return {a.y * b.z - b.y * a.z, a.z * b.x - b.z * a.x, a.x * b.y - b.x * a.y};
}
constexpr float kInf = std::numeric_limits<float>::infinity();

class SceneRng {
  public:
    explicit SceneRng(uint64_t seed) : state_(0), inc_((54ULL << 1) | 1ULL) {
        next_u32();
        state_ += seed;
        next_u32();
    }
    uint32_t next_u32() {
        const uint64_t old = state_;
        state_ = old * 6364136223846793005ULL + inc_;
        const uint32_t xs = static_cast<uint32_t>(((old >> 18) ^ old) >> 27);
        const uint32_t rot = static_cast<uint32_t>(old >> 59);
        return (xs >> rot) | (xs << ((32u - rot) & 31u));
    }
    float f32() { return static_cast<float>(next_u32() >> 8) * (1.0f / 16777216.0f); }
    float range(float lo, float hi) { return lo + (hi - lo) * f32(); }
  private:
    uint64_t state_, inc_;
};

wfpt_sphere make_sphere(Vec3 c, float r, uint32_t mat_idx, uint32_t mat_type) {
    wfpt_sphere s;
    s.center[0] = c.x; s.center[1] = c.y; s.center[2] = c.z; s.center[3] = 1.0f;
    s.radius = r; s.material_idx = mat_idx; s.material_type = mat_type; s._buffer = 0;
    return s;
// ... 585 lines not shown
        for (uint32_t i = 0; i < 256; ++i) {
            uint32_t c = i;
            for (int k = 0; k < 8; ++k) c = (c & 1u) ? 0xedb88320u ^ (c >> 1) : c >> 1;
            table[i] = c;
        }
        ready = true;
    }
    for (size_t i = 0; i < n; ++i) crc = table[(crc ^ p[i]) & 0xffu] ^ (crc >> 8);
    return crc;
}
static bool png_chunk(FILE *f, const char type[4], const std::vector<uint8_t> &data) {
    const uint32_t n = static_cast<uint32_t>(data.size());
    const uint8_t len[4] = {uint8_t(n >> 24), uint8_t(n >> 16), uint8_t(n >> 8), uint8_t(n)};
    uint32_t crc = png_crc(0xffffffffu, reinterpret_cast<const uint8_t *>(type), 4);
    crc = png_crc(crc, data.data(), data.size()) ^ 0xffffffffu;
    const uint8_t tail[4] = {uint8_t(crc >> 24), uint8_t(crc >> 16), uint8_t(crc >> 8), uint8_t(crc)};
    return std::fwrite(len, 1, 4, f) == 4 && std::fwrite(type, 1, 4, f) == 4 &&
           (data.empty() || std::fwrite(data.data(), 1, data.size(), f) == data.size()) && std::fwrite(tail, 1, 4, f) == 4;
}
int wfpt_write_png_rgb8(const char *path, const uint8_t *rgb, uint32_t width, uint32_t height) {
    if (!path || !rgb || width == 0 || height == 0) return WFPT_ERR_INVALID_ARGUMENT;
    const size_t row = 3 * static_cast<size_t>(width);
    std::vector<uint8_t> raw((row + 1) * height);
    for (uint32_t y = 0; y < height; ++y) {
        raw[y * (row + 1)] = 0;
        std::memcpy(&raw[y * (row + 1) + 1], rgb + y * row, row);
    }
    std::vector<uint8_t> z;
    z.reserve(raw.size() + raw.size() / 65535 * 5 + 16);
    z.push_back(0x78); z.push_back(0x01);
    uint32_t a = 1, b = 0;
    for (size_t off = 0; off < raw.size();) {
        const size_t n = std::min<size_t>(65535, raw.size() - off);
        z.push_back(off + n == raw.size() ? 1 : 0);
        z.push_back(uint8_t(n)); z.push_back(uint8_t(n >> 8));
        z.push_back(uint8_t(~n)); z.push_back(uint8_t((~n) >> 8));
        z.insert(z.end(), raw.begin() + off, raw.begin() + off + n);
        for (size_t i = off; i < off + n; ++i) { a = (a + raw[i]) % 65521u; b = (b + a) % 65521u; }
        off += n;
    }
    const uint32_t adler = (b << 16) | a;
    z.push_back(uint8_t(adler >> 24)); z.push_back(uint8_t(adler >> 16)); z.push_back(uint8_t(adler >> 8)); z.push_back(uint8_t(adler));
    FILE *f = std::fopen(path, "wb");
    if (!f) return WFPT_ERR_INVALID_ARGUMENT;
    static const uint8_t sig[8] = {0x89, 'P', 'N', 'G', 0x0d, 0x0a, 0x1a, 0x0a};
    std::vector<uint8_t> ihdr = {uint8_t(width >> 24), uint8_t(width >> 16), uint8_t(width >> 8), uint8_t(width),
                                 uint8_t(height >> 24), uint8_t(height >> 16), uint8_t(height >> 8), uint8_t(height),
                                 8, 2, 0, 0, 0};
    const bool ok = std::fwrite(sig, 1, 8, f) == 8 && png_chunk(f, "IHDR", ihdr) && png_chunk(f, "IDAT", z) && png_chunk(f, "IEND", {});
    std::fclose(f);
    return ok ? WFPT_OK : WFPT_ERR_INVALID_ARGUMENT;
}

}
```

wavefront_path_tracer_amd/csrc/wfpt_kernels.h:

```cpp
#pragma once
#include <hip/hip_runtime.h>
#include <stddef.h>
#include <stdint.h>

#include "wfpt.h"
#include "wfpt_bvh4.h"
#include "wfpt_device_math.h"

namespace wfpt {

#ifndef WFPT_CHUNK
#define WFPT_CHUNK 512
#endif
constexpr int kChunk = WFPT_CHUNK;
constexpr int kExtendThreads = kChunk;
constexpr int kExtendWaves = kExtendThreads / 64;
#ifndef WFPT_CONSUMER_THREADS
#define WFPT_CONSUMER_THREADS 256
#endif
constexpr int kConsumerThreads = WFPT_CONSUMER_THREADS;
constexpr int kScanThreads = 1024;
constexpr int kMaxRows = 64;
constexpr int kMaxTrailDepth = 63;
constexpr int kMaxBatch = 128;
constexpr int kClsMax = 8;
constexpr int kMaxBatchClassic = 64;

struct Stride32 {
    uint32_t v;
    __host__ __device__ operator size_t() const { return v; }
    __host__ __device__ Stride32 &operator=(size_t x) { v = static_cast<uint32_t>(x); return *this; }
};

struct RayQueue {
    float *base;
    uint32_t cap;
    __host__ __device__ float *ox() const { return base; }
    __host__ __device__ float *oy() const { return base + cap; }
    __host__ __device__ float *oz() const { return base + 2u * static_cast<size_t>(cap); }
    __host__ __device__ float *dx() const { return base + 3u * static_cast<size_t>(cap); }
    __host__ __device__ float *dy() const { return base + 4u * static_cast<size_t>(cap); }
    __host__ __device__ float *dz() const { return base + 5u * static_cast<size_t>(cap); }
    __host__ __device__ uint32_t *pixel() const { return reinterpret_cast<uint32_t *>(base + 6u * static_cast<size_t>(cap)); }
};

struct HitQueue {
    uint32_t *base;
    Stride32 plane;
    __host__ __device__ float *t() const { return reinterpret_cast<float *>(base); }
    __host__ __device__ uint32_t *prim() const { return base + static_cast<size_t>(plane); }
    __host__ __device__ uint32_t *ridx() const { return base + 2u * static_cast<size_t>(plane); }
};
struct MissQueue {
    uint32_t *base;
    Stride32 plane;
    __host__ __device__ uint32_t *ridx() const { return base; }
    __host__ __device__ float *dy() const { return reinterpret_cast<float *>(base + static_cast<size_t>(plane)); }
    __host__ __device__ uint32_t *pixel() const { return base + 2u * static_cast<size_t>(plane); }
    __host__ __device__ float *dx() const { return reinterpret_cast<float *>(base + 3u * static_cast<size_t>(plane)); }
    __host__ __device__ float *dz() const { return reinterpret_cast<float *>(base + 4u * static_cast<size_t>(plane)); }
// ... 122 lines not shown
    size_t mat_list_mstride;
    size_t chunk_mat_mstride;
    SceneDev scene;
};

struct ScanArgs {
    Batch batch;
    const uint32_t *chunk_hits, *chunk_miss;
    uint32_t *chunk_hit_base, *chunk_miss_base;
    Control *ctl;
    const uint32_t *n_in;
    uint32_t limit;
    uint32_t *first_seg;
    uint32_t fused;
    uint32_t miss_floor;
    uint32_t bounce;
};

constexpr int kBounceFirst = 0;
constexpr int kBounceMiddle = 1;
constexpr int kBounceLast = 2;
#ifndef WFPT_MISS_SEGS
#define WFPT_MISS_SEGS 16
#endif
constexpr int kMissSegsPerItem = WFPT_MISS_SEGS;
#ifndef WFPT_MISS_EVERY
#define WFPT_MISS_EVERY 0
#endif
constexpr uint32_t kMissEvery = WFPT_MISS_EVERY;

struct BounceArgs {
    Batch batch;
    unsigned long long *stamps;
    const float4 *rec_in;
    float4 *rec_out;
    const uint32_t *in_hits, *in_hit_base, *in_miss;
    const uint32_t *in_first_seg;
    uint32_t *out_hits, *out_miss;
    MissQueue mq_in, mq_out;
    float *image;
    Control *ctl;
    const CameraDev *camera;
    uint32_t gx, gy;
    uint32_t capacity;
    uint32_t rng_mode;
    uint32_t image_width;
    Tiling tile;
    SceneDev scene;
    const uint32_t *plan;
    uint32_t plan_seg_off, plan_miss_off;
    const uint2 *cls_table;
    const uint32_t *first_seg_cls;
    uint32_t *out_cls;
};

template <int K> struct ClsPack {
    static constexpr int kFields = K + 2, kWords = (kFields + 2) / 3;
};
constexpr int kBinClasses = 4;
static_assert(kBinClasses <= kClsMax && kChunk <= 1023, "a packed field must hold a segment's count");

struct ScanBinnedArgs {
    Batch batch;
    const uint32_t *chunk_hits, *chunk_miss, *chunk_cls;
    uint2 *cls_table;
    uint32_t *first_seg_cls;
    Control *ctl;
    const uint32_t *n_in;
    uint32_t limit, miss_floor, bounce;
};

struct PlanArgs {
    Batch batch;
    const Control *ctl;
    uint32_t *plan;
    uint32_t plan_seg_off, plan_miss_off;
    uint32_t last;
};

constexpr uint32_t kDenseMiss = 0xffffffffu, kDenseInactive = 0xfffffffeu;
#ifndef WFPT_TICKET_BLOCK
#define WFPT_TICKET_BLOCK 64
#endif
constexpr uint32_t kTicketBlock = WFPT_TICKET_BLOCK;
#ifndef WFPT_REFILL_IDLE_PRESHADED
#define WFPT_REFILL_IDLE_PRESHADED 24
#endif
#ifndef WFPT_REFILL_IDLE_FIRST_PRE
#define WFPT_REFILL_IDLE_FIRST_PRE 16
#endif
constexpr uint32_t kRefillIdlePreshaded = WFPT_REFILL_IDLE_PRESHADED, kRefillIdleFirstPre = WFPT_REFILL_IDLE_FIRST_PRE;

struct RefillArgs {
    Batch batch;
    unsigned long long *stamps;
    const float4 *rec_in;
    float4 *dense_out;
    const uint32_t *in_hits, *in_hit_base, *in_first_seg;
    float *image;
    Control *ctl;
    const CameraDev *camera;
    uint32_t gx, gy, capacity, rng_mode, image_width;
    Tiling tile;
    SceneDev scene;
};

// ... 167 lines not shown
}
__host__ __device__ inline uint32_t aov_channels(uint32_t which) { return which < 2u ? 3u : which < WFPT_AOV_COUNT ? 1u : 0u; }

constexpr uint32_t kMomentPlanes = 2;
__host__ __device__ inline float denoise_luma(float r, float g, float b) { return (0.2126f * r + 0.7152f * g) + 0.0722f * b; }
__host__ __device__ inline float variance_resolve(float s1, float s2, uint32_t n) {
    if (n == 0u) return 0.0f;
    const float nf = static_cast<float>(n);
    const float mu = s1 / nf;
    const float d = s2 / nf - mu * mu;
    return (d > 0.0f ? d : 0.0f) / nf;
}

struct DenoiseArgs {
    uint32_t width, height;
    uint32_t n;
    const float *accumulated;
    const float *aov_sums;
    const float *moments;
    Stride32 plane;
    float4 *guide_nz;
    float4 *guide_ag;
    const float4 *cv_in;
    float4 *cv_out;
    float *out;
    size_t out_floats;
    uint32_t step;
    float sigma_l, sigma_n, sigma_z, sigma_a2;
};
constexpr uint32_t kDenoiseTile = 16;

struct TemporalSlot {
    float4 *cl;
    float2 *m;
    float4 *nz;
    float2 *cm;
};
constexpr float kNoMotion = -1e30f;
struct TemporalArgs {
    const CameraDev *camera;
    float m[16];
    float pos_s[3];
    uint32_t has_sealed;
    float history_cap, depth_tolerance, normal_cos;
    TemporalSlot sealed;
    TemporalSlot live;
    float4 *motion;
};

hipError_t launch_generate(const GenerateArgs &a, hipStream_t s);
hipError_t launch_extend(const ExtendArgs &a, uint32_t grid, hipStream_t s, bool env_dirs = false);
hipError_t launch_scan(const ScanArgs &a, hipStream_t s);
hipError_t launch_bounce(const BounceArgs &a, int mode, uint32_t grid, hipStream_t s, bool env_dirs = false);
hipError_t launch_bounce_binned(const BounceArgs &a, int mode, uint32_t grid, hipStream_t s);
hipError_t launch_scan_binned(const ScanBinnedArgs &a, hipStream_t s);
hipError_t launch_plan(const PlanArgs &a, hipStream_t s);
hipError_t bounce_binned_blocks_per_cu(const SceneDev &scene, int *blocks);
hipError_t launch_refill(const RefillArgs &a, int mode, uint32_t grid, hipStream_t s);
hipError_t launch_shade_rays(const RefillArgs &a, uint32_t n_chunks, hipStream_t s);
hipError_t launch_generate_dense(const RefillArgs &a, hipStream_t s);
hipError_t launch_compact(const CompactArgs &a, uint32_t n_chunks, hipStream_t s, bool env_dirs = false);
hipError_t bounce_blocks_per_cu(const SceneDev &scene, int *blocks);
hipError_t launch_shade(const ShadeArgs &a, uint32_t grid, hipStream_t s);
hipError_t launch_miss(const MissArgs &a, uint32_t grid, hipStream_t s, const EnvDist *env = nullptr, const float *connected = nullptr,
                       bool weigh = false);
hipError_t launch_env_mis_weight(const EnvDist &env, const float *dirs3, float *out4, uint32_t n, hipStream_t s);
hipError_t launch_texture(const TextureArgs &a, uint32_t grid, hipStream_t s);
hipError_t launch_emission(const EmissionArgs &a, EmissionKind kind, uint32_t grid, hipStream_t s, float q = 1.0f);
hipError_t launch_mis_weight(const MisArgs &m, const float4 *shade_rec, const uint32_t *prim_em, const float *in8, float *out4, uint32_t n, hipStream_t s);
hipError_t launch_connect(const ConnectArgs &a, uint32_t grid, hipStream_t s, bool textured, bool envs = false, bool mis = false);
hipError_t launch_env_weights(const EnvDev &env, float *f, uint32_t *max_bits, hipStream_t s);
hipError_t launch_env_tables(const EnvDev &env, const float *f, float M, uint32_t *row, uint64_t *marg, hipStream_t s);
hipError_t connect_prepare(const SceneDev &scene);
hipError_t launch_accumulate(const AccumulateArgs &a, uint32_t grid, hipStream_t s);
hipError_t launch_accumulate_emission(const AccumulateArgs &a, const float *emitted, float *moments, size_t plane, uint32_t grid, hipStream_t s);
hipError_t launch_fill(float *p, float v, size_t n, hipStream_t s);
hipError_t launch_set_frame(Control *ctl, const wfpt_frame_buffer &f, hipStream_t s);
hipError_t launch_band_scatter(float *frame, const float *slab, size_t n_valid, size_t band_floats, uint32_t world, uint32_t rank, hipStream_t s);
hipError_t launch_rays_to_aos(const RayQueue &q, wfpt_ray *out, uint32_t n, hipStream_t s);
hipError_t launch_rays_from_aos(const RayQueue &q, const wfpt_ray *in, uint32_t n, hipStream_t s);
hipError_t launch_aov(const AovArgs &a, uint32_t grid, hipStream_t s, const EnvDev *env = nullptr, const TexScene *tex = nullptr);
hipError_t aov_prepare(const SceneDev &scene);
hipError_t launch_aov_resolve(const float *sums, size_t plane, uint32_t which, uint32_t n_samples, uint32_t *out, size_t n_words, hipStream_t s);
hipError_t launch_accumulate_moments(const AccumulateArgs &a, float *moments, size_t plane, uint32_t grid, hipStream_t s);
hipError_t launch_denoise_prepare(const DenoiseArgs &a, hipStream_t s);
hipError_t launch_denoise_atrous(const DenoiseArgs &a, hipStream_t s);
hipError_t launch_temporal_prepare(const DenoiseArgs &a, const TemporalArgs &t, hipStream_t s);
hipError_t launch_env_sample(const EnvDev &env, const float *dirs, float *rgb, size_t n, hipStream_t s);
hipError_t launch_tex_sample(const TexDev &tex, const float *uv, float *rgb, size_t n, hipStream_t s);
hipError_t launch_selftest_math(int op, const float *a, const float *b, float *out, size_t n, hipStream_t s);
hipError_t extend_blocks_per_cu(const SceneDev &scene, int *blocks);
uint32_t extend_lds_bytes(uint32_t n_nodes, uint32_t n_prims, uint32_t prim_kind, bool lds_scene);

}
```

wavefront_path_tracer_amd/csrc/wfpt_kernels.hip:

```cpp
#include "wfpt_kernels.h"
#include "wfpt_device_math.h"

namespace wfpt {

namespace {

constexpr float kPi = 3.1415927f;

__device__ __forceinline__ uint32_t lane_id() { return threadIdx.x & 63u; }
__device__ __forceinline__ uint32_t mbcnt(unsigned long long mask) {
    return __builtin_amdgcn_mbcnt_hi(static_cast<uint32_t>(mask >> 32),
                                     __builtin_amdgcn_mbcnt_lo(static_cast<uint32_t>(mask), 0u));
}
__device__ __forceinline__ uint32_t umin(uint32_t a, uint32_t b) { return a < b ? a : b; }
__device__ __forceinline__ uint32_t umax(uint32_t a, uint32_t b) { return a > b ? a : b; }
__device__ __forceinline__ uint32_t uniform(uint32_t v) { return __builtin_amdgcn_readfirstlane(v); }

#define WFPT_AS_LDS __attribute__((address_space(3)))
#define WFPT_AS_GLOBAL __attribute__((address_space(1)))
typedef float v4f_ __attribute__((ext_vector_type(4)));
__device__ __forceinline__ float4 load4_lds(const float4 *p) {
    const v4f_ v = *(const WFPT_AS_LDS v4f_ *)p;
    return make_float4(v.x, v.y, v.z, v.w);
}
// ... 1728 lines not shown
    const float4 *rec_in;
    const uint32_t *in_hit_base, *in_first_seg;
    const Control *ctl;
    float *image;
    const float4 *shade_rec;
    size_t qo, co;
    uint32_t capacity, rng_mode, image_width, prim_kind;
    Tiling tile;
};
template <bool SCATTER, bool WAVE_SMP, bool WAVE_H>
__device__ __forceinline__ void shade_record(const HitSource &s, float4 ra, float4 rb, uint32_t prim, uint32_t h, wfpt_frame_buffer fb, float &ox,
                                             float &oy, float &oz, float &dx, float &dy, float &dz, uint32_t &pixel_idx) {
    pixel_idx = __float_as_uint(ra.w);
    const float4 rec1 = s.shade_rec[3u * prim + 1u];
    float4 *px = pixel_of(s.image, local_pixel(pixel_idx, s.image_width, s.tile));
    const float4 thr = *px;
    if (SCATTER) {
        const float4 rec0 = s.shade_rec[3u * prim], rec2 = s.shade_rec[3u * prim + 2u];
        const uint32_t gx = WAVE_SMP ? uniform(s.ctl->shade_gx) : s.ctl->shade_gx;
        const uint32_t rng = shade_rng<WAVE_H>(s.rng_mode, h, gx, pixel_idx, fb);
        const float3_ ext = scatter(rng, {ra.x, ra.y, ra.z}, {rb.x, rb.y, rb.z}, rec0, rec1, __float_as_uint(rec2.x), s.prim_kind);
        ox = ra.x; oy = ra.y; oz = ra.z;
        dx = ext.x; dy = ext.y; dz = ext.z;
    }
    *px = make_float4(thr.x * rec1.x, thr.y * rec1.y, thr.z * rec1.z, thr.w);
}
#if WFPT_STAMPS
#define WFPT_SHADE_STAMPS_PARAM , unsigned long long *shade_stamps = nullptr
#else
#define WFPT_SHADE_STAMPS_PARAM
#endif
template <bool SCATTER>
__device__ __forceinline__ void shade_hit(const HitSource &s, uint32_t h, uint32_t n_hits, wfpt_frame_buffer fb, float &ox, float &oy,
                                          float &oz, float &dx, float &dy, float &dz, uint32_t &pixel_idx WFPT_SHADE_STAMPS_PARAM) {
    const uint32_t run = uniform(h / kChunk), n_runs = (n_hits + kChunk - 1) / kChunk;
    uint32_t lo = s.in_first_seg[s.co + run];
    uint32_t hi = run + 1 < n_runs ? s.in_first_seg[s.co + run + 1] : (umin(s.ctl->seg_n, s.capacity) + kChunk - 1) / kChunk - 1u;
    lo = uniform(lo); hi = uniform(hi);
    while (lo < hi) {
        const uint32_t mid = (lo + hi + 1u) >> 1;
        if (s.in_hit_base[s.co + mid] <= h) lo = mid; else hi = mid - 1u;
    }
    const size_t slot = s.qo + static_cast<size_t>(lo) * kChunk + (h - s.in_hit_base[s.co + lo]);
#if WFPT_STAMPS
    if (shade_stamps) { asm volatile("s_waitcnt vmcnt(0)" ::: "memory"); shade_stamps[0] = stamp_now(); }
#endif
    const float4 ra = s.rec_in[2u * slot], rb = s.rec_in[2u * slot + 1u];
#if WFPT_STAMPS
    if (shade_stamps) { asm volatile("s_waitcnt vmcnt(0)" ::: "memory"); shade_stamps[1] = stamp_now(); }
#endif
    shade_record<SCATTER, true, true>(s, ra, rb, __float_as_uint(rb.w), h, fb, ox, oy, oz, dx, dy, dz, pixel_idx);
}

struct TicketMap {
    uint32_t n_hit, every, n_mixed;
    __device__ __forceinline__ TicketMap(uint32_t n_hit_items, uint32_t n_items, bool mix) : n_hit(n_hit_items) {
        const uint32_t n_miss = n_items - n_hit_items;
        every = kMissEvery ? kMissEvery : uniform(umin(umax(n_hit_items / umax(n_miss, 1u), 1u), 62u)) + 1u;
        n_mixed = mix ? umin(n_miss, n_hit_items / (every - 1u)) : 0u;
    }
    __device__ __forceinline__ uint32_t item_of(uint32_t t) const {
        if (t < n_mixed * every) {
            const uint32_t k = t / every, r = t - k * every;
            return r == every - 1u ? n_hit + k : k * (every - 1u) + r;
        }
        const uint32_t u = t - n_mixed * every, rest_h = n_hit - n_mixed * (every - 1u);
        return u < rest_h ? n_mixed * (every - 1u) + u : n_hit + n_mixed + (u - rest_h);
    }
};

struct BounceLds {
    uint32_t *cnt;
    uint32_t *next;
    uint32_t *total;
    uint16_t *items_h;
    uint16_t *items_m;
    uint32_t *stack;
};
constexpr uint32_t kBounceMiscWords = 4u * kExtendWaves + 2u + 2u + kMaxBatch;
static_assert(kBounceMiscWords % 4u == 0, "the stack column area stays 16-byte aligned");

#define WFPT_MISS_ITEM(SMP, FIRST_SEG, N_SEGS)                                                                                         \
    {                                                                                                                                  \
        const uint32_t smp = (SMP), first_seg = (FIRST_SEG), n_segs = (N_SEGS);                                                        \
        const size_t qo = smp * a.batch.queue_stride, co = smp * a.batch.chunk_stride;                                                 \
        float *image = a.image + smp * a.batch.image_stride;                                                                           \
        for (uint32_t k = wave; k < kMissSegsPerItem; k += kExtendWaves) {                                                             \
            const uint32_t seg = first_seg + k;                                                                                        \
            if (seg >= n_segs) break;                                                                                                  \
            const uint32_t count = uniform(a.in_miss[co + seg]);                                                                       \
            for (uint32_t r = lane; r < count; r += 64u) {                                                                             \
                const size_t slot = qo + static_cast<size_t>(seg) * kChunk + r;                                                        \
                const float dy = a.mq_in.dy()[slot];                           \
                const uint32_t pixel_idx = a.mq_in.pixel()[slot];                                                                      \
                const float3_ c = sky(dy);                                                                                             \
                float4 *px = pixel_of(image, local_pixel(pixel_idx, a.image_width, a.tile));                                           \
                const float4 thr = *px;                                                                                                \
                *px = make_float4(thr.x * c.x, thr.y * c.y, thr.z * c.z, thr.w);                                         \
            }                                                                                                                          \
        }                                                                                                                              \
    }

#ifndef WFPT_BOUNCE_ATTR
#define WFPT_BOUNCE_ATTR __launch_bounds__(kExtendThreads, WFPT_EXTEND_MIN_WAVES)
#endif
template <int MODE, typename Trail, int PRIM, bool LDS_SCENE, bool EXACT, bool ENV = false>
// ... 53 lines not shown
            while (item >= first_m + uniform(L.items_m[smp_m])) first_m += uniform(L.items_m[smp_m++]);
            WFPT_MISS_ITEM(smp_m, (item - first_m) * kMissSegsPerItem, (uniform(umin(a.ctl[smp_m].seg_n, a.capacity)) + kChunk - 1) / kChunk);
            __syncthreads();
            ticket = uniform(L.next[buf]);
            item = tickets.item_of(ticket);
            iter += 1;
            continue;
        }
        WFPT_STAMP(t_item);
        while (item >= first_h + uniform(L.items_h[smp_h])) first_h += uniform(L.items_h[smp_h++]);
        const uint32_t smp = smp_h;
        const uint32_t seg_out = item - first_h;
        const uint32_t n = MODE == kBounceFirst ? umin(n_slots, a.capacity) : uniform(umin(a.ctl[smp].shade_n, a.capacity));
        const size_t qo = smp * a.batch.queue_stride, co = smp * a.batch.chunk_stride;
        float *image = a.image + smp * a.batch.image_stride;
        wfpt_frame_buffer fb = fb0;
        fb.frame += smp;

        const uint32_t h = seg_out * kChunk + threadIdx.x;
        bool live = h < n;
        float ox = 0, oy = 0, oz = 0, dx = 0, dy = 0, dz = 0;
        uint32_t pixel_idx = 0;
        if (MODE == kBounceFirst) {
            const TilePixel p = tile_pixel(uniform(h >> 6), h, a.gx, a.tile);
            live = live && p.x < fb.width && p.y < fb.height;
            if (live) {
                WFPT_START_PATH(pr, p, fb, image, ox = pr.ox; oy = pr.oy; oz = pr.oz; dx = pr.dx; dy = pr.dy; dz = pr.dz);
            }
        } else if (live) {
            const HitSource src{a.rec_in, a.in_hit_base, a.in_first_seg, a.ctl + smp, image, a.scene.shade_rec, qo, co,
                                a.capacity, a.rng_mode, a.image_width, a.scene.prim_kind, a.tile};
#if WFPT_STAMPS
            unsigned long long sst[2] = {t_item, t_item};
            shade_hit<TRACE>(src, h, n, fb, ox, oy, oz, dx, dy, dz, pixel_idx, sst);
            if (MODE == kBounceMiddle) { acc_search += sst[0] - t_item; acc_record += sst[1] - sst[0]; }
#else
            shade_hit<TRACE>(src, h, n, fb, ox, oy, oz, dx, dy, dz, pixel_idx);
#endif
        }
        if (!TRACE) {
            __syncthreads();
            ticket = uniform(L.next[buf]);
            item = tickets.item_of(ticket);
            iter += 1;
            continue;
        }
        WFPT_STAMP(t_trace);
#if WFPT_STAMPS
        uint32_t dbg[3] = {0, 0, 0};
#endif
        float t = 0.0f;
        uint32_t prim = 0;
        bool hit = false;
        if (live) WFPT_TRACE_ANY(g_nodes, L.stack, ox, oy, oz, dx, dy, dz);
        WFPT_STAMP(t_traced);
        const bool miss = live && !hit;
        const unsigned long long hit_mask = __ballot(hit), miss_mask = __ballot(miss);
        if (lane == 0) {
            L.cnt[(buf * 2 + 0) * kExtendWaves + wave] = static_cast<uint32_t>(__popcll(hit_mask));
            L.cnt[(buf * 2 + 1) * kExtendWaves + wave] = static_cast<uint32_t>(__popcll(miss_mask));
        }
        __syncthreads();
        WFPT_STAMP(t_synced);
        uint32_t hit_before, miss_before, hit_total, miss_total;
        wave_offsets(L.cnt + buf * 2u * kExtendWaves, wave, lane, hit_before, hit_total, miss_before, miss_total);
        const size_t seg = qo + static_cast<size_t>(seg_out) * kChunk;
        if (hit) {
            float4 *rec = a.rec_out + 2u * (seg + hit_before);
            const uint32_t rank = mbcnt(hit_mask);
            rec[2u * rank] = make_float4(ox + t * dx, oy + t * dy, oz + t * dz, __uint_as_float(pixel_idx));
            rec[2u * rank + 1u] = make_float4(dx, dy, dz, __uint_as_float(prim));
        }
        if (miss) {
            const size_t first = seg + miss_before;
            const uint32_t rank = mbcnt(miss_mask);
            (a.mq_out.dy() + first)[rank] = dy;
            (a.mq_out.pixel() + first)[rank] = pixel_idx;
            if (ENV) {
                (a.mq_out.dx() + first)[rank] = dx;
                (a.mq_out.dz() + first)[rank] = dz;
            }
        }
        if (threadIdx.x == 0) {
            a.out_hits[co + seg_out] = hit_total;
            a.out_miss[co + seg_out] = miss_total;
        }
#if WFPT_STAMPS
        if (MODE == kBounceMiddle) {
            asm volatile("s_waitcnt vmcnt(0)" ::: "memory");
            WFPT_STAMP(t_done);
            acc_cyc[0] += t_trace - t_item;
            acc_cyc[1] += t_traced - t_trace;
            acc_cyc[2] += t_synced - t_traced;
            acc_cyc[3] += t_done - t_synced;
            acc_cnt[0] += 1u;
            acc_cnt[1] += static_cast<uint32_t>(__popcll(__ballot(live)));
            uint32_t w_visits = dbg[0], w_leaves = dbg[1], l_visits = dbg[2];
            for (int d = 1; d < 64; d <<= 1) {
                w_visits = max(w_visits, static_cast<uint32_t>(__shfl_xor(w_visits, d, 64)));
                w_leaves = max(w_leaves, static_cast<uint32_t>(__shfl_xor(w_leaves, d, 64)));
                l_visits += static_cast<uint32_t>(__shfl_xor(l_visits, d, 64));
            }
            acc_cnt[2] += w_visits; acc_cnt[3] += w_leaves; acc_cnt[4] += l_visits;
        }
#endif
        ticket = uniform(L.next[buf]);
        item = tickets.item_of(ticket);
// ... 1597 lines not shown
    return misc + (sc.lds_scene ? scene_lds_bytes(sc.n_nodes, sc.n_spheres, sc.prim_kind) : kStackColumnBytes);
}
}

hipError_t bounce_blocks_per_cu(const SceneDev &scene, int *blocks) {
    const uint32_t bytes = bounce_dynamic_lds(scene, kBounceMiddle);
    for (bool exact : {false, true}) {
        const hipError_t e = allow_dynamic_lds(bytes, bounce_variant(scene, exact, kBounceFirst), bounce_variant(scene, exact, kBounceMiddle),
                                               bounce_variant(scene, exact, kBounceFirst, true), bounce_variant(scene, exact, kBounceMiddle, true));
        if (e != hipSuccess) return e;
    }
    return hipOccupancyMaxActiveBlocksPerMultiprocessor(blocks, bounce_variant(scene, scene.exact != 0, kBounceMiddle), kExtendThreads, bytes);
}

namespace {
uint32_t bounce_binned_lds(const SceneDev &sc, int mode) {
    const uint32_t misc = 4u * (2u * kExtendWaves * ClsPack<kBinClasses>::kWords + 2u + 2u) + ((sc.n_spheres + 15u) & ~15u);
    return mode == kBounceLast ? misc : misc + scene_lds_bytes(sc.n_nodes, sc.n_spheres, sc.prim_kind);
}
template <int MODE> struct BinnedK {
    template <typename Trail, int PRIM, bool LDS_SCENE, bool EXACT> static BounceFn get() { return bounce_binned_kernel<MODE, Trail, PRIM, EXACT, kBinClasses>; }
};
BounceFn bounce_binned_variant(const SceneDev &sc, bool exact, int mode) {
    if (mode == kBounceLast) return bounce_binned_kernel<kBounceLast, uint32_t, 0, false, kBinClasses>;
    return mode == kBounceFirst ? pick_variant<BinnedK<kBounceFirst>>(sc, exact, true) : pick_variant<BinnedK<kBounceMiddle>>(sc, exact, true);
}
}

hipError_t bounce_binned_blocks_per_cu(const SceneDev &scene, int *blocks) {
    const uint32_t bytes = bounce_binned_lds(scene, kBounceMiddle);
    for (bool exact : {false, true}) {
        const hipError_t e = allow_dynamic_lds(bytes, bounce_binned_variant(scene, exact, kBounceFirst), bounce_binned_variant(scene, exact, kBounceMiddle));
        if (e != hipSuccess) return e;
    }
    return hipOccupancyMaxActiveBlocksPerMultiprocessor(blocks, bounce_binned_variant(scene, scene.exact != 0, kBounceMiddle), kExtendThreads, bytes);
}

hipError_t launch_bounce_binned(const BounceArgs &a, int mode, uint32_t grid, hipStream_t s) {
    if (grid == 0) return hipSuccess;
    hipLaunchKernelGGL(bounce_binned_variant(a.scene, a.scene.exact != 0, mode), dim3(grid), dim3(kExtendThreads), bounce_binned_lds(a.scene, mode), s, a);
    return hipGetLastError();
}

hipError_t launch_scan_binned(const ScanBinnedArgs &a, hipStream_t s) {
    hipLaunchKernelGGL(scan_binned_kernel<kBinClasses>, dim3(a.batch.n), dim3(kScanThreads), 0, s, a);
    return hipGetLastError();
}

hipError_t launch_plan(const PlanArgs &a, hipStream_t s) {
    hipLaunchKernelGGL(plan_kernel<kBinClasses>, dim3(1), dim3(kPlanThreads), 0, s, a);
    return hipGetLastError();
}

hipError_t launch_bounce(const BounceArgs &a, int mode, uint32_t grid, hipStream_t s, bool env_dirs) {
    if (grid == 0) return hipSuccess;
    hipLaunchKernelGGL(bounce_variant(a.scene, a.scene.exact != 0, mode, env_dirs), dim3(grid), dim3(kExtendThreads), bounce_dynamic_lds(a.scene, mode), s, a);
    return hipGetLastError();
}

namespace {
constexpr uint32_t kRefillLdsFixed = 4u * (2u * kMaxBatch + 4u + kStack4Lds * kExtendThreads);
}

hipError_t launch_refill(const RefillArgs &a, int mode, uint32_t grid, hipStream_t s) {
    if (grid == 0) return hipSuccess;
    using Fn = void (*)(RefillArgs);
    Fn fn;
    if (mode == kBounceFirst) fn = a.scene.prim_kind == 0 ? refill_kernel<kBounceFirst, 0> : refill_kernel<kBounceFirst, 1>;
    else fn = a.scene.prim_kind == 0 ? refill_kernel<kBounceMiddle, 0> : refill_kernel<kBounceMiddle, 1>;
    hipLaunchKernelGGL(fn, dim3(grid), dim3(kExtendThreads), kRefillLdsFixed + 64u * a.scene.tile_n, s, a);
    return hipGetLastError();
}

hipError_t launch_shade_rays(const RefillArgs &a, uint32_t n_chunks, hipStream_t s) {
    if (n_chunks == 0) return hipSuccess;
    hipLaunchKernelGGL(shade_rays_kernel, dim3(n_chunks, a.batch.n), dim3(kExtendThreads), 0, s, a);
    return hipGetLastError();
}

hipError_t launch_generate_dense(const RefillArgs &a, hipStream_t s) {
    const uint32_t n = a.gx * a.gy * 64u < a.capacity ? a.gx * a.gy * 64u : a.capacity;
    if (n == 0) return hipSuccess;
    hipLaunchKernelGGL(generate_dense_kernel, dim3((n + 255u) / 256u, a.batch.n), dim3(256), 0, s, a);
    return hipGetLastError();
}

hipError_t launch_compact(const CompactArgs &a, uint32_t n_chunks, hipStream_t s, bool env_dirs) {
    if (n_chunks == 0) return hipSuccess;
    hipLaunchKernelGGL(env_dirs ? compact_kernel<true> : compact_kernel<false>, dim3(n_chunks, a.batch.n), dim3(kExtendThreads), 0, s, a);
    return hipGetLastError();
}

hipError_t launch_generate(const GenerateArgs &a, hipStream_t s) {
    const uint32_t n = a.gx * a.gy * 64u;
    if (n == 0) return hipSuccess;
    hipLaunchKernelGGL(generate_rays_kernel, dim3((n + 255u) / 256u, a.batch.n), dim3(256), 0, s, a);
    return hipGetLastError();
}

hipError_t launch_extend(const ExtendArgs &a, uint32_t grid, hipStream_t s, bool env_dirs) {
    if (grid == 0) return hipSuccess;
    hipLaunchKernelGGL(extend_variant(a.scene, a.scene.exact != 0, a.has_inactive != 0, env_dirs), dim3(grid), dim3(kExtendThreads), a.scene.lds_bytes, s, a);
    return hipGetLastError();
}

hipError_t launch_scan(const ScanArgs &a, hipStream_t s) {
// ... 244 lines not shown
```

wfpt-sys/src/lib.rs:

```rust
#![allow(non_camel_case_types)]

use std::os::raw::{c_char, c_int, c_void};

pub const WFPT_INACTIVE_PIXEL: u32 = 0xffffffff;
pub const WFPT_MAX_TEXTURES: u32 = 64;
pub const WFPT_COMM_UNIQUE_ID_BYTES: u32 = 128;

pub const WFPT_OK: c_int = 0;
pub const WFPT_ERR_INVALID_ARGUMENT: c_int = -1;
pub const WFPT_ERR_HIP: c_int = -2;
pub const WFPT_ERR_OUT_OF_MEMORY: c_int = -3;
pub const WFPT_ERR_UNSUPPORTED: c_int = -4;
pub const WFPT_ERR_NO_DEVICE: c_int = -5;

pub const WFPT_STAGE_GENERATE_RAYS: c_int = 0;
pub const WFPT_STAGE_EXTEND: c_int = 1;
pub const WFPT_STAGE_SHADE: c_int = 2;
pub const WFPT_STAGE_MISS: c_int = 3;
pub const WFPT_STAGE_ACCUMULATE: c_int = 4;
pub const WFPT_STAGE_SHADE_LAMBERTIAN: c_int = 5;
pub const WFPT_STAGE_SHADE_METAL: c_int = 6;
pub const WFPT_STAGE_SHADE_DIELECTRIC: c_int = 7;
pub const WFPT_STAGE_SCAN: c_int = 8;
pub const WFPT_STAGE_BOUNCE_FIRST: c_int = 9;
pub const WFPT_STAGE_BOUNCE: c_int = 10;
pub const WFPT_STAGE_BOUNCE_LAST: c_int = 11;
pub const WFPT_STAGE_COMPACT: c_int = 12;
pub const WFPT_STAGE_COUNT: c_int = 13;

pub const WFPT_RNG_DISPATCH: c_int = 0;
pub const WFPT_RNG_PIXEL: c_int = 1;

pub const WFPT_LOOP_STAGES: c_int = 0;
pub const WFPT_LOOP_FUSED: c_int = 1;
pub const WFPT_LOOP_FUSED_BINNED: c_int = 2;
pub const WFPT_LOOP_REFILL: c_int = 3;

pub const WFPT_AOV_ALBEDO: c_int = 0;
pub const WFPT_AOV_NORMAL: c_int = 1;
pub const WFPT_AOV_DEPTH: c_int = 2;
pub const WFPT_AOV_COVERAGE: c_int = 3;
pub const WFPT_AOV_PRIM_ID: c_int = 4;
pub const WFPT_AOV_MATERIAL_ID: c_int = 5;
pub const WFPT_AOV_COUNT: c_int = 6;

pub const WFPT_TEMPORAL_COLOR: c_int = 0;
pub const WFPT_TEMPORAL_MOMENTS: c_int = 1;
pub const WFPT_TEMPORAL_LENGTH: c_int = 2;
pub const WFPT_TEMPORAL_MOTION: c_int = 3;

pub const WFPT_TEXTURE_BILINEAR: c_int = 0;
pub const WFPT_TEXTURE_NEAREST: c_int = 1;

pub const WFPT_FLAG_SPLIT_SHADE: u32 = 1 << 0;
pub const WFPT_FLAG_NO_GRAPH: u32 = 1 << 1;
pub const WFPT_FLAG_UNFUSED: u32 = 1 << 2;
pub const WFPT_FLAG_BINARY_BVH: u32 = 1 << 3;
pub const WFPT_FLAG_NO_REFILL: u32 = 1 << 4;
pub const WFPT_FLAG_NO_LDS_SCENE: u32 = 1 << 5;
pub const WFPT_FLAG_EXACT_TRAVERSAL: u32 = 1 << 6;
pub const WFPT_FLAG_NO_BINNING: u32 = 1 << 7;
pub const WFPT_FLAG_BINNING: u32 = 1 << 8;
pub const WFPT_FLAG_AOV: u32 = 1 << 10;
pub const WFPT_FLAG_DENOISE: u32 = 1 << 11;
pub const WFPT_FLAG_ENVIRONMENT: u32 = 1 << 12;
pub const WFPT_FLAG_TEXTURES: u32 = 1 << 13;
pub const WFPT_FLAG_EMISSION: u32 = 1 << 14;
pub const WFPT_FLAG_NEE: u32 = 1 << 15;
pub const WFPT_FLAG_ENV_NEE: u32 = 1 << 16;
pub const WFPT_FLAG_MIS: u32 = 1 << 17;
pub const WFPT_FLAG_ENV_MIS: u32 = 1 << 18;

#[repr(C)]
#[derive(Copy, Clone, Debug, Default)]
pub struct wfpt_sphere {
    pub center: [f32; 4],
    pub radius: f32,
    pub material_idx: u32,
    pub material_type: u32,
    pub _buffer: u32,
}

#[repr(C)]
#[derive(Copy, Clone, Debug, Default)]
pub struct wfpt_material {
    pub albedo: [f32; 4],
    pub fuzz: f32,
    pub refract_index: f32,
    pub material_type: u32,
    pub _buffer: u32,
}

#[repr(C)]
#[derive(Copy, Clone, Debug, Default)]
pub struct wfpt_bvh_node {
    pub aabb_min: [f32; 3],
    pub left_first: u32,
    pub aabb_max: [f32; 3],
    pub prim_count: u32,
}

#[repr(C)]
#[derive(Copy, Clone, Debug, Default)]
pub struct wfpt_triangle {
    pub v0: [f32; 3],
    pub material_idx: u32,
    pub e1: [f32; 3],
    pub material_type: u32,
    pub e2: [f32; 3],
    pub _pad: u32,
}

#[repr(C)]
#[derive(Copy, Clone, Debug, Default)]
pub struct wfpt_gpu_camera {
    pub position: [f32; 4],
    pub pitch: f32,
    pub yaw: f32,
    pub defocus_radius: f32,
    pub focus_distance: f32,
}

#[repr(C)]
#[derive(Copy, Clone, Debug, Default)]
// ... 153 lines not shown
    pub fn wfpt_sample_environment(ctx: *mut wfpt_ctx, dirs: *const f32, n: usize, rgb_out: *mut f32) -> c_int;
    pub fn wfpt_texture_params_default(p: *mut wfpt_texture_params);
    pub fn wfpt_set_texture(ctx: *mut wfpt_ctx, slot: u32, rgb: *const f32, w: u32, h: u32, p: *const wfpt_texture_params) -> c_int;
    pub fn wfpt_clear_texture(ctx: *mut wfpt_ctx, slot: u32) -> c_int;
    pub fn wfpt_bind_texture(ctx: *mut wfpt_ctx, material_idx: u32, slot: i32) -> c_int;
    pub fn wfpt_set_triangle_uvs(ctx: *mut wfpt_ctx, uv6: *const f32, n_rows: u32) -> c_int;
    pub fn wfpt_sample_texture(ctx: *mut wfpt_ctx, slot: u32, uv: *const f32, n: usize, rgb_out: *mut f32) -> c_int;
    pub fn wfpt_texture_timing_ms(ctx: *mut wfpt_ctx, ms_total: *mut f32, launches: *mut u32) -> c_int;
    pub fn wfpt_set_emission(ctx: *mut wfpt_ctx, material_idx: u32, rgb: *const f32) -> c_int;
    pub fn wfpt_get_emission(ctx: *mut wfpt_ctx, material_idx: u32, rgb: *mut f32) -> c_int;
    pub fn wfpt_clear_emission(ctx: *mut wfpt_ctx) -> c_int;
    pub fn wfpt_emission_timing_ms(ctx: *mut wfpt_ctx, ms_total: *mut f32, launches: *mut u32) -> c_int;
    pub fn wfpt_nee_light_count(ctx: *mut wfpt_ctx) -> c_int;
    pub fn wfpt_nee_timing_ms(ctx: *mut wfpt_ctx, ms_total: *mut f32, launches: *mut u32) -> c_int;
    pub fn wfpt_sample_lights(ctx: *mut wfpt_ctx, in9: *const f32, n: usize, out8: *mut f32) -> c_int;
    pub fn wfpt_set_environment_share(ctx: *mut wfpt_ctx, share: f32) -> c_int;
    pub fn wfpt_environment_share(ctx: *const wfpt_ctx) -> f32;
    pub fn wfpt_read_environment_distribution(ctx: *mut wfpt_ctx, row_wh: *mut u32, marg_h: *mut u64) -> c_int;
    pub fn wfpt_sample_environment_light(ctx: *mut wfpt_ctx, in10: *const f32, n: usize, out8: *mut f32) -> c_int;
    pub fn wfpt_sample_lights_mis(ctx: *mut wfpt_ctx, in9: *const f32, n: usize, out12: *mut f32) -> c_int;
    pub fn wfpt_mis_hit_weight(ctx: *mut wfpt_ctx, in8: *const f32, n: usize, out4: *mut f32) -> c_int;
    pub fn wfpt_sample_environment_light_mis(ctx: *mut wfpt_ctx, in10: *const f32, n: usize, out12: *mut f32) -> c_int;
    pub fn wfpt_env_mis_miss_weight(ctx: *mut wfpt_ctx, dirs3: *const f32, n: usize, out4: *mut f32) -> c_int;
    pub fn wfpt_n_pixels(ctx: *const wfpt_ctx) -> u32;
    pub fn wfpt_ray_capacity(ctx: *const wfpt_ctx) -> u32;
    pub fn wfpt_read_accumulated(ctx: *mut wfpt_ctx, rgb: *mut f32, n_floats: usize) -> c_int;
    pub fn wfpt_read_image(ctx: *mut wfpt_ctx, rgb: *mut f32, n_floats: usize) -> c_int;
    pub fn wfpt_copy_accumulated_to_device(ctx: *mut wfpt_ctx, device_ptr: *mut c_void, n_bytes: usize) -> c_int;
    pub fn wfpt_comm_unique_id(id128: *mut c_void) -> c_int;
    pub fn wfpt_comm_init(ctx: *mut wfpt_ctx, id128: *const c_void, rank: c_int, world: c_int) -> c_int;
    pub fn wfpt_gather_accumulated(ctx: *mut wfpt_ctx) -> c_int;
    pub fn wfpt_gather_accumulated_timed(ctx: *mut wfpt_ctx, ms: *mut f32) -> c_int;
    pub fn wfpt_read_gathered(ctx: *mut wfpt_ctx, rgb: *mut f32, n_floats: usize) -> c_int;
    pub fn wfpt_comm_destroy(ctx: *mut wfpt_ctx) -> c_int;
    pub fn wfpt_read_rays(ctx: *mut wfpt_ctx, rays: *mut wfpt_ray, n: u32) -> c_int;
    pub fn wfpt_read_extension_rays(ctx: *mut wfpt_ctx, rays: *mut wfpt_ray, n: u32) -> c_int;
    pub fn wfpt_read_hits(ctx: *mut wfpt_ctx, hits: *mut wfpt_hit_payload, n: u32) -> c_int;
    pub fn wfpt_read_misses(ctx: *mut wfpt_ctx, ray_indices: *mut u32, n: u32) -> c_int;
    pub fn wfpt_write_rays(ctx: *mut wfpt_ctx, rays: *const wfpt_ray, n: u32) -> c_int;
    pub fn wfpt_read_bounce_table(ctx: *mut wfpt_ctx, rows4: *mut u32, max_rows: u32, n_rows: *mut u32) -> c_int;
    pub fn wfpt_read_totals(ctx: *mut wfpt_ctx, totals: *mut u64) -> c_int;
    pub fn wfpt_read_wavefront_totals(ctx: *mut wfpt_ctx, rows3: *mut u64, max_rows: u32, n_rows: *mut u32) -> c_int;
    pub fn wfpt_device_info(device: c_int, compute_units: *mut u32, memory_clock_khz: *mut u32, memory_bus_width_bits: *mut u32, total_memory_bytes: *mut u64) -> c_int;
    pub fn wfpt_tonemap_rgb8(accumulated: *const f32, n_pixels: u32, n_samples: u32, rgb: *mut u8);
    pub fn wfpt_save_ppm(ctx: *mut wfpt_ctx, path: *const c_char) -> c_int;
    pub fn wfpt_save_pfm(ctx: *mut wfpt_ctx, path: *const c_char) -> c_int;
    pub fn wfpt_save_png(ctx: *mut wfpt_ctx, path: *const c_char) -> c_int;
    pub fn wfpt_write_png_rgb8(path: *const c_char, rgb: *const u8, width: u32, height: u32) -> c_int;
    pub fn wfpt_selftest_math(device: c_int, op: c_int, a: *const f32, b: *const f32, out: *mut f32, n: usize) -> c_int;
    pub fn wfpt_debug_extend_blocks_per_cu(device: c_int, lds_bytes: u32) -> c_int;
    pub fn wfpt_debug_read_stamps(ctx: *mut wfpt_ctx, out: *mut u64, reset: c_int) -> c_int;
    pub fn wfpt_debug_read_stamps_ex(ctx: *mut wfpt_ctx, which: c_int, out: *mut u64, reset: c_int) -> c_int;
    pub fn wfpt_debug_bvh4(nodes: *const wfpt_bvh_node, n_nodes: u32, counts: *mut u32) -> c_int;
    pub fn wfpt_build_info() -> *const c_char;
}
```

Before: 23530.

## Add per-tile primary-ray BVH leaf lists to skip traversal on first bounce

Builds, for each 8x8 screen tile, a conservative frustum bundle covering the tile's pixel rays, including the lens. It then records up to 16 BVH leaves that the bundle can reach. The first-bounce kernel receives these lists so primary rays can test only the candidate leaves instead of traversing the whole BVH. Lists are built lazily after the first kept batch and invalidated on camera or scene change. This adds a build kernel, buffer memory and extra conservative-bound logic, and falls back to full traversal when a tile needs more leaves than the cap.

```diff
diff --git a/include/wfpt.h b/include/wfpt.h
--- a/include/wfpt.h
+++ b/include/wfpt.h
@@ -145,7 +145,8 @@
     WFPT_FLAG_NEE = 1u << 15         ,
     WFPT_FLAG_ENV_NEE = 1u << 16     ,
     WFPT_FLAG_MIS = 1u << 17         ,
-    WFPT_FLAG_ENV_MIS = 1u << 18
+    WFPT_FLAG_ENV_MIS = 1u << 18,
+    WFPT_FLAG_NO_TILE_LISTS = 1u << 19
 };
 
 #define WFPT_INACTIVE_PIXEL 0xffffffffu
@@ -398,6 +399,13 @@
 int wfpt_debug_read_stamps(wfpt_ctx *ctx, uint64_t out[16], int reset);
 int wfpt_debug_read_stamps_ex(wfpt_ctx *ctx, int which, uint64_t out[16], int reset);
 int wfpt_debug_bvh4(const wfpt_bvh_node *nodes, uint32_t n_nodes, uint32_t counts[4]);
+#define WFPT_TILE_LIST_CAP 16u
+#define WFPT_TILE_NO_LIST 0xffffffffu
+int wfpt_tile_lists_host(const float *nodes_ch, uint32_t n_nodes, const wfpt_gpu_camera *camera, const float inv_proj[16], const float view[16],
+                         uint32_t width, uint32_t height, uint32_t tile_rank, uint32_t tile_world, uint32_t *records, uint32_t n_tiles);
+int wfpt_debug_nodes_ch(const wfpt_bvh_node *nodes, uint32_t n_nodes, const wfpt_gpu_camera *camera, float *nodes_ch);
+int wfpt_debug_read_tile_lists(wfpt_ctx *ctx, uint32_t *records, uint32_t *n_tiles);
+int wfpt_tile_lists_timing_ms(wfpt_ctx *ctx, float *ms_last, uint32_t *builds);
 const char *wfpt_build_info(void);
 
 #ifdef __cplusplus
diff --git a/wavefront_path_tracer_amd/__init__.py b/wavefront_path_tracer_amd/__init__.py
--- a/wavefront_path_tracer_amd/__init__.py
+++ b/wavefront_path_tracer_amd/__init__.py
@@ -7,7 +7,7 @@
 
 __all__ = ["SPP", "SPF", "Scene", "BVHTree", "Camera", "CameraController", "ProjectionMatrix", "GPUFrameBuffer",
            "RenderParameters", "RenderProgress", "Kernel", "PathTracer", "WfptError", "workgroup_size_64",
-           "RNG_DISPATCH", "RNG_PIXEL", "FLAG_SPLIT_SHADE", "FLAG_NO_GRAPH", "FLAG_UNFUSED", "FLAG_BINARY_BVH", "FLAG_NO_REFILL", "FLAG_NO_LDS_SCENE", "FLAG_EXACT_TRAVERSAL", "FLAG_NO_BINNING", "FLAG_BINNING", "FLAG_AOV", "AOVS", "FLAG_DENOISE", "DENOISE_DEFAULTS", "FLAG_ENVIRONMENT", "load_environment", "FLAG_TEXTURES", "MAX_TEXTURES", "load_texture", "FLAG_EMISSION", "FLAG_NEE", "FLAG_ENV_NEE", "FLAG_MIS", "FLAG_ENV_MIS", "TEMPORAL_DEFAULTS", "TEMPORAL_OUTPUTS", "STAGES", "lib", "build",
+           "RNG_DISPATCH", "RNG_PIXEL", "FLAG_SPLIT_SHADE", "FLAG_NO_GRAPH", "FLAG_UNFUSED", "FLAG_BINARY_BVH", "FLAG_NO_REFILL", "FLAG_NO_LDS_SCENE", "FLAG_EXACT_TRAVERSAL", "FLAG_NO_BINNING", "FLAG_BINNING", "FLAG_AOV", "AOVS", "FLAG_DENOISE", "DENOISE_DEFAULTS", "FLAG_ENVIRONMENT", "load_environment", "FLAG_TEXTURES", "MAX_TEXTURES", "load_texture", "FLAG_EMISSION", "FLAG_NEE", "FLAG_ENV_NEE", "FLAG_MIS", "FLAG_ENV_MIS", "FLAG_NO_TILE_LISTS", "TILE_LIST_CAP", "TILE_NO_LIST", "tile_lists_host", "nodes_ch", "TEMPORAL_DEFAULTS", "TEMPORAL_OUTPUTS", "STAGES", "lib", "build",
            "tonemap_rgb8", "selftest_math", "device_count"]
 
 SPP = 10
@@ -26,6 +26,8 @@
 FLAG_ENV_NEE = 1 << 16
 FLAG_MIS = 1 << 17
 FLAG_ENV_MIS = 1 << 18
+FLAG_NO_TILE_LISTS = 1 << 19
+TILE_LIST_CAP, TILE_NO_LIST = 16, 0xFFFFFFFF
 FLAG_DENOISE = 1 << 11
 DENOISE_DEFAULTS = {"iterations": 5, "sigma_luminance": 4.0, "sigma_normal": 128.0, "sigma_depth": 1.0, "sigma_albedo": 0.5}
 TEMPORAL_DEFAULTS = {**DENOISE_DEFAULTS, "history_cap": 32.0, "depth_tolerance": 0.05, "normal_cos": 0.9}
@@ -320,6 +322,10 @@
         "wfpt_mis_hit_weight": (i32, [vp, vp, sz, vp]),
         "wfpt_sample_environment_light_mis": (i32, [vp, vp, sz, vp]),
         "wfpt_env_mis_miss_weight": (i32, [vp, vp, sz, vp]),
+        "wfpt_tile_lists_host": (i32, [vp, u32, vp, vp, vp, u32, u32, u32, u32, vp, u32]),
+        "wfpt_debug_nodes_ch": (i32, [vp, u32, vp, vp]),
+        "wfpt_debug_read_tile_lists": (i32, [vp, vp, C.POINTER(u32)]),
+        "wfpt_tile_lists_timing_ms": (i32, [vp, C.POINTER(f32), C.POINTER(u32)]),
     }
     for name, (res, args) in sig.items():
         fn = getattr(L, name)
@@ -342,6 +348,27 @@
 
 def _p(a):
     return a.ctypes.data_as(C.c_void_p)
+
+
+def nodes_ch(nodes, gpu_camera):
+    out = np.zeros((len(nodes), 8), np.float32)
+    st = lib().wfpt_debug_nodes_ch(_p(nodes), len(nodes), _p(gpu_camera), _p(out))
+    if st != 0:
+        raise WfptError(st, lib().wfpt_last_error(None).decode())
+    return out
+
+
+def tile_lists_host(nodes, gpu_camera, inv_proj, view, width, height, tile_rank=0, tile_world=1):
+    ch = nodes_ch(nodes, gpu_camera)
+    gx, bands = (width + 7) // 8, (height + 7) // 8
+    gy = (bands - tile_rank + tile_world - 1) // tile_world if bands > tile_rank else 0
+    out = np.zeros((gx * gy, TILE_LIST_CAP), np.uint32)
+    inv_proj, view = np.ascontiguousarray(inv_proj, np.float32), np.ascontiguousarray(view, np.float32)
+    st = lib().wfpt_tile_lists_host(_p(ch), len(nodes), _p(gpu_camera), _p(inv_proj), _p(view), width, height, tile_rank, tile_world,
+                                    _p(out), gx * gy)
+    if st != 0:
+        raise WfptError(st, "wfpt_tile_lists_host: invalid argument")
+    return out
 
 
 def device_count():
@@ -1113,6 +1140,20 @@
         self._check(lib().wfpt_denoise_to_device(self.handle, C.byref(p), C.c_void_p(tensor.data_ptr()), 4 * n))
         return tensor
 
+    def read_tile_lists(self):
+        n = C.c_uint32(0)
+        self._check(lib().wfpt_debug_read_tile_lists(self.handle, None, C.byref(n)))
+        if n.value == 0:
+            return None
+        out = np.zeros((n.value, TILE_LIST_CAP), np.uint32)
+        self._check(lib().wfpt_debug_read_tile_lists(self.handle, _p(out), C.byref(n)))
+        return out
+
+    def tile_lists_timing(self):
+        ms, n = C.c_float(0.0), C.c_uint32(0)
+        self._check(lib().wfpt_tile_lists_timing_ms(self.handle, C.byref(ms), C.byref(n)))
+        return float(ms.value), int(n.value)
+
     def denoise_timing(self):
         ms, n = C.c_float(0.0), C.c_uint32(0)
         self._check(lib().wfpt_denoise_timing_ms(self.handle, C.byref(ms), C.byref(n)))
diff --git a/wavefront_path_tracer_amd/_build.py b/wavefront_path_tracer_amd/_build.py
--- a/wavefront_path_tracer_amd/_build.py
+++ b/wavefront_path_tracer_amd/_build.py
@@ -7,7 +7,7 @@
 CSRC = os.path.join(PKG_DIR, "csrc")
 LIB_PATH = os.path.join(PKG_DIR, "libwfpt.so")
 SOURCES = ["wfpt_kernels.hip", "wfpt_api.hip", "wfpt_bvh_build.hip", "wfpt_host.cpp"]
-HEADERS = [os.path.join(CSRC, "wfpt_kernels.h"), os.path.join(CSRC, "wfpt_bvh4.h"), os.path.join(CSRC, "wfpt_device_math.h"),
+HEADERS = [os.path.join(CSRC, "wfpt_kernels.h"), os.path.join(CSRC, "wfpt_bvh4.h"), os.path.join(CSRC, "wfpt_device_math.h"), os.path.join(CSRC, "wfpt_tile_lists.h"),
            os.path.join(ROOT, "include", "wfpt.h")]
 FLAGS = ["--offload-arch=gfx950", "-O3", "-std=c++17", "-fPIC", "-shared", "-ffp-contract=off",
          "-fhip-fp32-correctly-rounded-divide-sqrt", "-fno-fast-math", "-Wall", "-Wno-unused-function"]
diff --git a/wavefront_path_tracer_amd/csrc/wfpt_api.hip b/wavefront_path_tracer_amd/csrc/wfpt_api.hip
--- a/wavefront_path_tracer_amd/csrc/wfpt_api.hip
+++ b/wavefront_path_tracer_amd/csrc/wfpt_api.hip
@@ -242,6 +242,14 @@
     uint32_t accumulate_grid = 0;
     uint32_t progress_frame = 0, accumulated_samples = 0;
     bool dev_frame_valid = false;
+    DeviceBuffer<uint32_t> tile_lists;
+    bool tile_lists_valid = false;
+    bool tl_cleared = true;
+    bool tl_kept = false;
+    EventPair tl_ev;
+    bool tl_pending = false;
+    float tl_ms = 0.0f;
+    uint32_t tl_builds = 0;
 
     std::map<uint32_t, Graph> graphs;
 
@@ -634,6 +642,10 @@
     if (c->rec_dense.get() && !c->scene.exact) return WFPT_LOOP_REFILL;
     return use_binned(c) ? WFPT_LOOP_FUSED_BINNED : WFPT_LOOP_FUSED;
 }
+const uint4 *tile_lists_of(const wfpt_ctx *c) {
+    const bool keeps = c->tile_lists.get() && loop_of(c) == WFPT_LOOP_FUSED && c->scene.lds_scene && !c->scene.exact && c->scene.nodes_ch;
+    return keeps ? reinterpret_cast<const uint4 *>(c->tile_lists.get()) : nullptr;
+}
 uint32_t bounce_grid(const wfpt_ctx *c, uint32_t n) {
     const uint64_t items = (static_cast<uint64_t>(c->n_chunks_max) * 5u / 4u + 1u) * n;
     return static_cast<uint32_t>(std::min<uint64_t>(items, static_cast<uint64_t>(c->cus) * c->bounce_blocks_per_cu));
@@ -682,7 +694,11 @@
     const hipStream_t st = c->stream.get();
     const uint32_t grid = bounce_grid(c, nb);
     const EnvDev *env = env_of(c);
-    WFPT_HIP(c, timed(WFPT_STAGE_BOUNCE_FIRST, [&] { return launch_bounce(bounce_args(c, 1, 0, nb), kBounceFirst, grid, st, env != nullptr); }));
+    WFPT_HIP(c, timed(WFPT_STAGE_BOUNCE_FIRST, [&] {
+                 BounceArgs a = bounce_args(c, 1, 0, nb);
+                 a.tile_lists = tile_lists_of(c);
+                 return launch_bounce(a, kBounceFirst, grid, st, env != nullptr);
+             }));
     for (uint32_t b = 0; b < c->p.max_wavefronts; ++b) {
         const int par = static_cast<int>(b & 1u);
         const bool last = b + 1 >= c->p.max_wavefronts;
@@ -816,8 +832,19 @@
     c->tp_read_ok = false;
 }
 
+int drop_tile_lists(wfpt_ctx *c) {
+    c->tile_lists_valid = false;
+    c->tl_kept = false;
+    if (!c->tile_lists.get() || c->tl_cleared) return WFPT_OK;
+    WFPT_HIP(c, hipSetDevice(c->device));
+    WFPT_HIP(c, hipMemsetAsync(c->tile_lists.get(), 0xff, sizeof(uint32_t) * c->tile_lists.size(), c->stream.get()));
+    c->tl_cleared = true;
+    return WFPT_OK;
+}
+
 int scene_changed(wfpt_ctx *c) {
     c->graphs.clear();
+    if (int r = drop_tile_lists(c); r != WFPT_OK) return r;
     c->hit_rec_valid = false;
     drop_history(c);
     return wfpt_reset_progress(c);
@@ -829,6 +856,7 @@
     c->progress_frame += nb;
     c->accumulated_samples += nb;
     c->last_slot = nb - 1;
+    c->tl_kept = true;
 }
 
 int ensure_device_frame(wfpt_ctx *c) {
@@ -839,9 +867,38 @@
     return WFPT_OK;
 }
 
+#ifndef WFPT_TILE_LISTS_EAGER
+#define WFPT_TILE_LISTS_EAGER 0
+#endif
+int ensure_tile_lists(wfpt_ctx *c, bool now = false) {
+    if (c->tile_lists_valid || !tile_lists_of(c)) return WFPT_OK;
+    if (!now && !WFPT_TILE_LISTS_EAGER && !c->tl_kept) return WFPT_OK;
+    TileListArgs a{};
+    a.nodes_ch = c->scene.nodes_ch;
+    a.n_nodes = c->scene.n_nodes;
+    a.camera = c->camera.get();
+    a.gx = c->tiles_x;
+    a.gy = c->tiles_y_local;
+    a.width = c->width;
+    a.height = c->height;
+    a.tile = c->tile;
+    a.records = c->tile_lists.get();
+    if (static_cast<size_t>(a.gx) * a.gy * kTileListCap > c->tile_lists.size()) return fail(c, WFPT_ERR_INVALID_ARGUMENT, "tile lists: the viewport exceeds the table");
+    WFPT_HIP(c, c->tl_ev.create());
+    WFPT_HIP(c, hipEventRecord(c->tl_ev.start.get(), c->stream.get()));
+    WFPT_HIP(c, launch_tile_lists(a, c->stream.get()));
+    WFPT_HIP(c, hipEventRecord(c->tl_ev.stop.get(), c->stream.get()));
+    c->tl_pending = true;
+    c->tl_builds += 1;
+    c->tile_lists_valid = true;
+    c->tl_cleared = false;
+    return WFPT_OK;
+}
+
 int render_batch(wfpt_ctx *c, uint32_t nb) {
     WFPT_HIP(c, hipSetDevice(c->device));
     if (int r = ensure_device_frame(c); r != WFPT_OK) return r;
+    if (int r = ensure_tile_lists(c); r != WFPT_OK) return r;
     if (c->p.flags & WFPT_FLAG_NO_GRAPH) {
         if (int r = enqueue_batch(c, nullptr, nb); r != WFPT_OK) return r;
     } else {
@@ -1397,6 +1454,10 @@
             CREATE_HIP(c->f_chunk_miss[k].alloc_zeroed(counts, st));
         }
         CREATE_HIP(c->first_seg.alloc_zeroed(counts, st));
+        if (!(c->p.flags & WFPT_FLAG_NO_TILE_LISTS)) {
+            CREATE_HIP(c->tile_lists.alloc(static_cast<size_t>(c->capacity / 64u) * kTileListCap));
+            CREATE_HIP(hipMemsetAsync(c->tile_lists.get(), 0xff, sizeof(uint32_t) * c->tile_lists.size(), st));
+        }
         if (c->bin_capable) {
             for (int k = 0; k < 2; ++k) CREATE_HIP(c->f_cls[k].alloc_zeroed(counts * ClsPack<kBinClasses>::kWords, st));
             CREATE_HIP(c->cls_table.alloc_zeroed(counts * kBinClasses, st));
@@ -1477,6 +1538,7 @@
         p.tile_world = chunks;
         p.max_pixels = 0;
         p.flags &= ~static_cast<uint32_t>(WFPT_FLAG_AOV | WFPT_FLAG_DENOISE | WFPT_FLAG_ENVIRONMENT | WFPT_FLAG_TEXTURES | WFPT_FLAG_EMISSION | WFPT_FLAG_NEE | WFPT_FLAG_ENV_NEE | WFPT_FLAG_MIS | WFPT_FLAG_ENV_MIS);
+        p.flags |= WFPT_FLAG_NO_TILE_LISTS;
         if (bands_of(h, k, chunks) == 0) continue;
         g_last_status = WFPT_ERR_HIP;
         wfpt_ctx *c = create_impl(&p, spheres, triangles, n_prims, materials, n_materials, nodes, n_nodes, camera, inv_proj, view);
@@ -1554,6 +1616,7 @@
     WFPT_HIP(c, hipMemcpy(c->camera.get(), &cam, sizeof cam, hipMemcpyHostToDevice));
     if (int r = wfpt_reset_progress(c); r != WFPT_OK) return r;
     c->graphs.clear();
+    if (int r = drop_tile_lists(c); r != WFPT_OK) return r;
     c->h_camera = *camera;
     std::memcpy(c->h_inv_proj, inv_proj, sizeof c->h_inv_proj);
     std::memcpy(c->h_view, view, sizeof c->h_view);
@@ -1779,6 +1842,7 @@
     while (n_samples > 0) {
         const uint32_t nb = std::min(n_samples, c->batch_max);
         if (int r = ensure_device_frame(c); r != WFPT_OK) return r;
+        if (int r = ensure_tile_lists(c); r != WFPT_OK) return r;
         std::vector<EventRec> ev;
         if (int r = enqueue_batch(c, &ev, nb); r != WFPT_OK) return r;
         WFPT_HIP(c, hipStreamSynchronize(c->stream.get()));
@@ -2557,6 +2621,42 @@
     return WFPT_OK;
 }
 
+int wfpt_debug_nodes_ch(const wfpt_bvh_node *nodes, uint32_t n_nodes, const wfpt_gpu_camera *camera, float *nodes_ch) {
+    if (!nodes || !camera || !nodes_ch || n_nodes == 0) return fail(nullptr, WFPT_ERR_INVALID_ARGUMENT, "wfpt_debug_nodes_ch: null or empty argument");
+    float reach[3], extent[3];
+    camera_reach(*camera, reach);
+    std::vector<float4> ch;
+    if (!build_nodes_ch(nodes, n_nodes, reach, ch, extent)) return fail(nullptr, WFPT_ERR_UNSUPPORTED, "wfpt_debug_nodes_ch: a box is not finite");
+    std::memcpy(nodes_ch, ch.data(), sizeof(float4) * ch.size());
+    return WFPT_OK;
+}
+
+int wfpt_debug_read_tile_lists(wfpt_ctx *c, uint32_t *records, uint32_t *n_tiles) {
+    if (!c || !n_tiles) return fail(c, WFPT_ERR_INVALID_ARGUMENT, "wfpt_debug_read_tile_lists: null argument");
+    WFPT_HIP(c, hipSetDevice(c->device));
+    const uint32_t have = *n_tiles, tiles = tile_lists_of(c) ? c->tiles_x * c->tiles_y_local : 0u;
+    *n_tiles = tiles;
+    if (tiles == 0 || !records) return WFPT_OK;
+    if (have < tiles) return fail(c, WFPT_ERR_INVALID_ARGUMENT, "wfpt_debug_read_tile_lists: the buffer holds fewer records than the context has tiles");
+    if (int r = ensure_tile_lists(c, true); r != WFPT_OK) return r;
+    WFPT_HIP(c, hipMemcpyAsync(records, c->tile_lists.get(), sizeof(uint32_t) * kTileListCap * tiles, hipMemcpyDeviceToHost, c->stream.get()));
+    WFPT_HIP(c, hipStreamSynchronize(c->stream.get()));
+    return WFPT_OK;
+}
+
+int wfpt_tile_lists_timing_ms(wfpt_ctx *c, float *ms_last, uint32_t *builds) {
+    if (!c) return fail(c, WFPT_ERR_INVALID_ARGUMENT, "wfpt_tile_lists_timing_ms: null context");
+    if (c->tl_pending) {
+        WFPT_HIP(c, hipSetDevice(c->device));
+        WFPT_HIP(c, hipEventSynchronize(c->tl_ev.stop.get()));
+        WFPT_HIP(c, hipEventElapsedTime(&c->tl_ms, c->tl_ev.start.get(), c->tl_ev.stop.get()));
+        c->tl_pending = false;
+    }
+    if (ms_last) *ms_last = c->tl_ms;
+    if (builds) *builds = c->tl_builds;
+    return WFPT_OK;
+}
+
 int wfpt_debug_extend_blocks_per_cu(int device, uint32_t lds_bytes) {
     int n_dev = 0;
     if (hipGetDeviceCount(&n_dev) != hipSuccess || device < 0 || device >= n_dev)
diff --git a/wavefront_path_tracer_amd/csrc/wfpt_host.cpp b/wavefront_path_tracer_amd/csrc/wfpt_host.cpp
--- a/wavefront_path_tracer_amd/csrc/wfpt_host.cpp
+++ b/wavefront_path_tracer_amd/csrc/wfpt_host.cpp
@@ -1,5 +1,6 @@
 #include "wfpt.h"
 #include "wfpt_bvh4.h"
+#include "wfpt_tile_lists.h"
 
 #include <algorithm>
 #include <cmath>
@@ -691,4 +692,36 @@
     return ok ? WFPT_OK : WFPT_ERR_INVALID_ARGUMENT;
 }
 
-}
+int wfpt_tile_lists_host(const float *nodes_ch, uint32_t n_nodes, const wfpt_gpu_camera *camera, const float inv_proj[16], const float view[16],
+                         uint32_t width, uint32_t height, uint32_t tile_rank, uint32_t tile_world, uint32_t *records, uint32_t n_tiles) {
+    if (!nodes_ch || !camera || !inv_proj || !view || !records || n_nodes == 0 || width == 0 || height == 0 || tile_world == 0 || tile_rank >= tile_world)
+        return WFPT_ERR_INVALID_ARGUMENT;
+    const uint32_t gx = (width + 7u) / 8u, bands = (height + 7u) / 8u;
+    const uint32_t gy = bands > tile_rank ? (bands - tile_rank + tile_world - 1u) / tile_world : 0u;
+    if (static_cast<uint64_t>(gx) * gy != n_tiles) return WFPT_ERR_INVALID_ARGUMENT;
+    auto word = [&](uint32_t i, int k) { uint32_t u; std::memcpy(&u, nodes_ch + 8u * static_cast<size_t>(i) + k, 4); return u; };
+    const bool root_leaf = word(0, 7) != 0u;
+    for (uint32_t tile = 0; tile < n_tiles; ++tile) {
+        uint32_t *rec = records + static_cast<size_t>(tile) * wfpt::kTileListCap;
+        uint32_t x0, y0, count = 0;
+        wfpt::tile_origin(tile, gx, tile_rank, tile_world, x0, y0);
+        const wfpt::TileBundle b = wfpt::tile_bundle(*camera, inv_proj, view, x0, y0, width, height);
+        bool list = b.ok != 0u && !root_leaf;
+        for (uint32_t k = 0; k < wfpt::kTileListCap; ++k) rec[k] = 0u;
+        for (uint32_t i = 0; i < n_nodes && list; ++i) {
+            const uint32_t w = wfpt::tile_leaf_word(i, word(i, 3), word(i, 7));
+            if (w == 0u) continue;
+            const float *n = nodes_ch + 8u * static_cast<size_t>(i);
+            if (w != wfpt::kTileNoList && !wfpt::tile_bundle_reaches(b, n[0], n[1], n[2], n[4], n[5], n[6])) continue;
+            if (w == wfpt::kTileNoList || count == wfpt::kTileListCap) list = false;
+            else rec[count++] = w;
+        }
+        if (!list) {
+            for (uint32_t k = 0; k < wfpt::kTileListCap; ++k) rec[k] = 0u;
+            rec[0] = wfpt::kTileNoList;
+        }
+    }
+    return WFPT_OK;
+}
+
+}
diff --git a/wavefront_path_tracer_amd/csrc/wfpt_kernels.h b/wavefront_path_tracer_amd/csrc/wfpt_kernels.h
--- a/wavefront_path_tracer_amd/csrc/wfpt_kernels.h
+++ b/wavefront_path_tracer_amd/csrc/wfpt_kernels.h
@@ -6,6 +6,7 @@
 #include "wfpt.h"
 #include "wfpt_bvh4.h"
 #include "wfpt_device_math.h"
+#include "wfpt_tile_lists.h"
 
 namespace wfpt {
 
@@ -234,6 +235,17 @@
     const uint2 *cls_table;
     const uint32_t *first_seg_cls;
     uint32_t *out_cls;
+    const uint4 *tile_lists;
+};
+
+struct TileListArgs {
+    const float4 *nodes_ch;
+    uint32_t n_nodes;
+    const CameraDev *camera;
+    uint32_t gx, gy;
+    uint32_t width, height;
+    Tiling tile;
+    uint32_t *records;
 };
 
 template <int K> struct ClsPack {
@@ -507,6 +519,7 @@
 hipError_t launch_extend(const ExtendArgs &a, uint32_t grid, hipStream_t s, bool env_dirs = false);
 hipError_t launch_scan(const ScanArgs &a, hipStream_t s);
 hipError_t launch_bounce(const BounceArgs &a, int mode, uint32_t grid, hipStream_t s, bool env_dirs = false);
+hipError_t launch_tile_lists(const TileListArgs &a, hipStream_t s);
 hipError_t launch_bounce_binned(const BounceArgs &a, int mode, uint32_t grid, hipStream_t s);
 hipError_t launch_scan_binned(const ScanBinnedArgs &a, hipStream_t s);
 hipError_t launch_plan(const PlanArgs &a, hipStream_t s);
diff --git a/wavefront_path_tracer_amd/csrc/wfpt_kernels.hip b/wavefront_path_tracer_amd/csrc/wfpt_kernels.hip
--- a/wavefront_path_tracer_amd/csrc/wfpt_kernels.hip
+++ b/wavefront_path_tracer_amd/csrc/wfpt_kernels.hip
@@ -1804,6 +1804,65 @@
     shade_record<SCATTER, true, true>(s, ra, rb, __float_as_uint(rb.w), h, fb, ox, oy, oz, dx, dy, dz, pixel_idx);
 }
 
+typedef uint32_t v4u_ __attribute__((ext_vector_type(4)));
+#define WFPT_AS_CONSTANT __attribute__((address_space(4)))
+template <int PRIM>
+__device__ __forceinline__ bool trace_tile_list(const uint4 *record, uint32_t w0, const float4 *prim_geom, float ox, float oy, float oz, float dx,
+                                                float dy, float dz, float &t_out, uint32_t &prim_out) {
+    const float a = (dx * dx + dy * dy) + dz * dz;
+    float nearest = 1e30f;
+    uint32_t best = 0xffffffffu, best_leaf = 0;
+    const WFPT_AS_CONSTANT v4u_ *rec = (const WFPT_AS_CONSTANT v4u_ *)reinterpret_cast<uintptr_t>(record);
+    uint32_t w = w0;
+    for (uint32_t q = 0; q < kTileListCap / 4u && w != 0u; ++q) {
+        const v4u_ four = rec[q];
+        const uint32_t ws[4] = {four.x, four.y, four.z, four.w};
+#pragma unroll
+        for (int k = 0; k < 4; ++k) {
+            w = ws[k];
+            if (w == 0u) break;
+            visit_leaf<PRIM>(prim_geom, w & 0xffffu, w >> 16, w, ox, oy, oz, dx, dy, dz, a, nearest, best, best_leaf);
+        }
+    }
+    leaf_box_verdict<PRIM>(prim_geom, best_leaf & 0xffffu, best_leaf >> 16, false, ox, oy, oz, dx, dy, dz, nearest, best);
+    t_out = nearest;
+    prim_out = best;
+    return nearest < 1e30f;
+}
+
+constexpr int kTileListThreads = 256;
+__global__ __launch_bounds__(kTileListThreads) void tile_lists_kernel(TileListArgs a) {
+    const uint32_t lane = lane_id();
+    const uint32_t tile = uniform(blockIdx.x * (kTileListThreads / 64u) + (threadIdx.x >> 6));
+    if (tile >= a.gx * a.gy) return;
+    uint32_t *rec = a.records + static_cast<size_t>(tile) * kTileListCap;
+    uint32_t x0, y0;
+    tile_origin(tile, a.gx, a.tile.rank, a.tile.world, x0, y0);
+    const CameraDev &cam = *a.camera;
+    const TileBundle b = tile_bundle(cam.cam, cam.inv_proj, cam.view, x0, y0, a.width, a.height);
+    bool list = b.ok != 0u && __float_as_uint(a.nodes_ch[1].w) == 0u;
+    uint32_t count = 0;
+    for (uint32_t base = 0; base < a.n_nodes && list; base += 64u) {
+        const uint32_t i = base + lane;
+        uint32_t w = 0u;
+        if (i < a.n_nodes) {
+            const float4 c = a.nodes_ch[2u * i], h = a.nodes_ch[2u * i + 1u];
+            w = tile_leaf_word(i, __float_as_uint(c.w), __float_as_uint(h.w));
+            if (w != 0u && w != kTileNoList && !tile_bundle_reaches(b, c.x, c.y, c.z, h.x, h.y, h.z)) w = 0u;
+        }
+        const unsigned long long mask = __ballot(w != 0u);
+        const uint32_t slot = count + mbcnt(mask);
+        if (__ballot(w == kTileNoList) != 0ull) list = false;
+        if (w != 0u && slot < kTileListCap) rec[slot] = w;
+        count += static_cast<uint32_t>(__popcll(mask));
+        if (count > kTileListCap) list = false;
+    }
+    if (lane < kTileListCap) {
+        if (!list) rec[lane] = lane == 0u ? kTileNoList : 0u;
+        else if (lane >= count) rec[lane] = 0u;
+    }
+}
+
 struct TicketMap {
     uint32_t n_hit, every, n_mixed;
     __device__ __forceinline__ TicketMap(uint32_t n_hit_items, uint32_t n_items, bool mix) : n_hit(n_hit_items) {
@@ -1963,7 +2022,22 @@
         float t = 0.0f;
         uint32_t prim = 0;
         bool hit = false;
-        if (live) WFPT_TRACE_ANY(g_nodes, L.stack, ox, oy, oz, dx, dy, dz);
+        if (MODE == kBounceFirst && LDS_SCENE && !EXACT) {
+            const uint4 *record = nullptr;
+            uint32_t w0 = kTileNoList;
+            if (a.tile_lists) {
+                record = a.tile_lists + (kTileListCap / 4u) * uniform(h >> 6);
+                w0 = uniform(*reinterpret_cast<const uint32_t *>(record));
+            }
+            if (w0 == kTileNoList) {
+                if (live) WFPT_TRACE_ANY(g_nodes, L.stack, ox, oy, oz, dx, dy, dz);
+            } else if (live) {
+                prim = kHandOver;
+                if (!far_origin(a.scene, ox, oy, oz)) hit = trace_tile_list<PRIM>(record, w0, s_geom, ox, oy, oz, dx, dy, dz, t, prim);
+                if (prim == kHandOver)
+                    hit = retrace_reference<Trail, PRIM, uint16_t>(g_nodes, s_geom, s_parent, ox, oy, oz, dx, dy, dz, a.scene.n_nodes, t, prim);
+            }
+        } else if (live) WFPT_TRACE_ANY(g_nodes, L.stack, ox, oy, oz, dx, dy, dz);
         WFPT_STAMP(t_traced);
         const bool miss = live && !hit;
         const unsigned long long hit_mask = __ballot(hit), miss_mask = __ballot(miss);
@@ -3667,6 +3741,13 @@
     return hipGetLastError();
 }
 
+hipError_t launch_tile_lists(const TileListArgs &a, hipStream_t s) {
+    const uint32_t tiles = a.gx * a.gy, per_block = kTileListThreads / 64u;
+    if (tiles == 0) return hipSuccess;
+    hipLaunchKernelGGL(tile_lists_kernel, dim3((tiles + per_block - 1u) / per_block), dim3(kTileListThreads), 0, s, a);
+    return hipGetLastError();
+}
+
 hipError_t launch_bounce(const BounceArgs &a, int mode, uint32_t grid, hipStream_t s, bool env_dirs) {
     if (grid == 0) return hipSuccess;
     hipLaunchKernelGGL(bounce_variant(a.scene, a.scene.exact != 0, mode, env_dirs), dim3(grid), dim3(kExtendThreads), bounce_dynamic_lds(a.scene, mode), s, a);
diff --git a/wavefront_path_tracer_amd/csrc/wfpt_tile_lists.h b/wavefront_path_tracer_amd/csrc/wfpt_tile_lists.h
--- /dev/null
+++ b/wavefront_path_tracer_amd/csrc/wfpt_tile_lists.h
@@ -0,0 +1,145 @@
+#pragma once
+#include <stdint.h>
+
+#include "wfpt.h"
+
+#if defined(__HIP__)
+#define WFPT_TL_FN __host__ __device__ inline
+#else
+#define WFPT_TL_FN inline
+#endif
+
+namespace wfpt {
+
+constexpr uint32_t kTileListCap = 16;
+constexpr uint32_t kTileNoList = 0xffffffffu;
+constexpr float kTilePixelPad = 0.0625f;
+constexpr float kTileSlop = 3.8146973e-6f;
+
+struct TileBundle {
+    float ax, ay, az;
+    float n[4][3];
+    float fx, fy, fz;
+    float rw;
+    float inv_df;
+    float a1;
+    uint32_t ok;
+};
+
+WFPT_TL_FN bool tl_finite(float v) { return __builtin_fabsf(v) < 1e30f; }
+
+WFPT_TL_FN TileBundle tile_bundle(const wfpt_gpu_camera &cam, const float *inv_proj, const float *view, uint32_t x0, uint32_t y0, uint32_t width,
+                                  uint32_t height) {
+    TileBundle b;
+    b.ok = 0u;
+    const bool lens = cam.defocus_radius > 0.0f;
+    const float fw = static_cast<float>(width), fh = static_cast<float>(height);
+    const float px[2] = {(static_cast<float>(x0) - 1.0f) - kTilePixelPad, (static_cast<float>(x0) + 8.0f) + kTilePixelPad};
+    const float py[2] = {(static_cast<float>(y0) - 1.0f) - kTilePixelPad, (static_cast<float>(y0) + 8.0f) + kTilePixelPad};
+    float w[4][3];
+    bool ok = width <= 16384u && height <= 16384u && view[3] == 0.0f && view[7] == 0.0f && view[11] == 0.0f && view[15] == 1.0f;
+    float sign_w = 0.0f, sign_z = 0.0f;
+    for (int k = 0; k < 4; ++k) {
+        const float cx = px[(k == 1 || k == 2) ? 1 : 0], cy = py[k >= 2 ? 1 : 0];
+        float ndc_x = cx / fw;
+        float ndc_y = 1.0f - cy / fh;
+        ndc_x = 2.0f * ndc_x - 1.0f;
+        ndc_y = 2.0f * ndc_y - 1.0f;
+        const float qx = ((inv_proj[0] * ndc_x + inv_proj[4] * ndc_y) + inv_proj[8] * 1.0f) + inv_proj[12] * 1.0f;
+        const float qy = ((inv_proj[1] * ndc_x + inv_proj[5] * ndc_y) + inv_proj[9] * 1.0f) + inv_proj[13] * 1.0f;
+        const float qz = ((inv_proj[2] * ndc_x + inv_proj[6] * ndc_y) + inv_proj[10] * 1.0f) + inv_proj[14] * 1.0f;
+        const float qw = ((inv_proj[3] * ndc_x + inv_proj[7] * ndc_y) + inv_proj[11] * 1.0f) + inv_proj[15] * 1.0f;
+        float gx = qx / qw, gy = qy / qw, gz = qz / qw;
+        ok = ok && tl_finite(gx) && tl_finite(gy) && tl_finite(gz) && qw != 0.0f && (k == 0 || (qw > 0.0f) == (sign_w > 0.0f));
+        sign_w = k == 0 ? qw : sign_w;
+        if (lens) {
+            ok = ok && gz != 0.0f && (k == 0 || (gz > 0.0f) == (sign_z > 0.0f));
+            sign_z = k == 0 ? gz : sign_z;
+            const float tf = cam.focus_distance / gz;
+            gx = tf * gx;
+            gy = tf * gy;
+            gz = tf * gz;
+        }
+        w[k][0] = ((view[0] * gx + view[4] * gy) + view[8] * gz) + view[12] * 0.0f;
+        w[k][1] = ((view[1] * gx + view[5] * gy) + view[9] * gz) + view[13] * 0.0f;
+        w[k][2] = ((view[2] * gx + view[6] * gy) + view[10] * gz) + view[14] * 0.0f;
+        ok = ok && tl_finite(w[k][0]) && tl_finite(w[k][1]) && tl_finite(w[k][2]);
+    }
+    b.ax = lens ? view[12] : cam.position[0];
+    b.ay = lens ? view[13] : cam.position[1];
+    b.az = lens ? view[14] : cam.position[2];
+    b.a1 = (__builtin_fabsf(b.ax) + __builtin_fabsf(b.ay)) + __builtin_fabsf(b.az);
+    ok = ok && tl_finite(b.a1);
+    const float c0x = view[0], c0y = view[1], c0z = view[2], c1x = view[4], c1y = view[5], c1z = view[6];
+    float fx = c0y * c1z - c0z * c1y, fy = c0z * c1x - c0x * c1z, fz = c0x * c1y - c0y * c1x;
+    const float fl = __builtin_sqrtf((fx * fx + fy * fy) + fz * fz);
+    ok = ok && fl > 0.0f && tl_finite(fl);
+    float inv = 1.0f / fl;
+    if (((fx * w[0][0] + fy * w[0][1]) + fz * w[0][2]) < 0.0f) inv = -inv;
+    fx = fx * inv;
+    fy = fy * inv;
+    fz = fz * inv;
+    b.fx = fx; b.fy = fy; b.fz = fz;
+    float df = 1e30f;
+    for (int k = 0; k < 4; ++k) {
+        const float d = (fx * w[k][0] + fy * w[k][1]) + fz * w[k][2];
+        df = d < df ? d : df;
+    }
+    ok = ok && df > 0.0f;
+    b.inv_df = 1.0f / df;
+    if (lens) {
+        const float n0 = (c0x * c0x + c0y * c0y) + c0z * c0z, n1 = (c1x * c1x + c1y * c1y) + c1z * c1z;
+        const float s2 = (n0 > n1 ? n0 : n1) + __builtin_fabsf((c0x * c1x + c0y * c1y) + c0z * c1z);
+        b.rw = (cam.defocus_radius * __builtin_sqrtf(s2)) * 1.000001f;
+        ok = ok && tl_finite(b.rw);
+    } else {
+        b.rw = 0.0f;
+    }
+    for (int k = 0; k < 4; ++k) {
+        const float *u = w[k], *v = w[(k + 1) & 3], *t = w[(k + 2) & 3];
+        float nx = u[1] * v[2] - u[2] * v[1], ny = u[2] * v[0] - u[0] * v[2], nz = u[0] * v[1] - u[1] * v[0];
+        const float nl = __builtin_sqrtf((nx * nx + ny * ny) + nz * nz);
+        ok = ok && nl > 0.0f && tl_finite(nl);
+        float ninv = 1.0f / nl;
+        if (((nx * t[0] + ny * t[1]) + nz * t[2]) < 0.0f) ninv = -ninv;
+        b.n[k][0] = nx * ninv;
+        b.n[k][1] = ny * ninv;
+        b.n[k][2] = nz * ninv;
+        ok = ok && tl_finite(b.n[k][0]) && tl_finite(b.n[k][1]) && tl_finite(b.n[k][2]);
+    }
+    b.ok = ok ? 1u : 0u;
+    return b;
+}
+
+WFPT_TL_FN bool tile_bundle_reaches(const TileBundle &b, float cx, float cy, float cz, float hx, float hy, float hz) {
+    const float dx = cx - b.ax, dy = cy - b.ay, dz = cz - b.az;
+    const float mag = ((((__builtin_fabsf(dx) + __builtin_fabsf(dy)) + __builtin_fabsf(dz)) + ((hx + hy) + hz)) + b.a1) +
+                      ((((__builtin_fabsf(cx) + __builtin_fabsf(cy)) + __builtin_fabsf(cz))) + b.rw);
+    const float slop = kTileSlop * mag;
+    if (!(mag < 1e30f)) return true;
+    const float depth = ((b.fx * dx + b.fy * dy) + b.fz * dz) + ((__builtin_fabsf(b.fx) * hx + __builtin_fabsf(b.fy) * hy) + __builtin_fabsf(b.fz) * hz);
+    if (depth + slop < 0.0f) return false;
+    const float u1 = (depth + slop) * b.inv_df - 1.0f;
+    const float rho = b.rw * ((u1 > 1.0f ? u1 : 1.0f) * 1.000001f) + slop;
+    bool reach = true;
+    for (int k = 0; k < 4; ++k) {
+        const float nx = b.n[k][0], ny = b.n[k][1], nz = b.n[k][2];
+        const float s = ((nx * dx + ny * dy) + nz * dz) + ((__builtin_fabsf(nx) * hx + __builtin_fabsf(ny) * hy) + __builtin_fabsf(nz) * hz);
+        reach = reach && !(s + rho < 0.0f);
+    }
+    return reach;
+}
+
+WFPT_TL_FN void tile_origin(uint32_t tile, uint32_t gx, uint32_t rank, uint32_t world, uint32_t &x0, uint32_t &y0) {
+    const uint32_t wx = tile % gx, wy = tile / gx;
+    x0 = wx * 8u;
+    y0 = (wy * world + rank) * 8u;
+}
+
+WFPT_TL_FN uint32_t tile_leaf_word(uint32_t i, uint32_t left_first, uint32_t prim_count) {
+    if (i == 1u || prim_count == 0u) return 0u;
+    if (prim_count >= 0xffffu || left_first > 0xffffu) return kTileNoList;
+    return left_first | (prim_count << 16);
+}
+
+}
diff --git a/wfpt-sys/src/lib.rs b/wfpt-sys/src/lib.rs
--- a/wfpt-sys/src/lib.rs
+++ b/wfpt-sys/src/lib.rs
@@ -5,6 +5,8 @@
 pub const WFPT_INACTIVE_PIXEL: u32 = 0xffffffff;
 pub const WFPT_MAX_TEXTURES: u32 = 64;
 pub const WFPT_COMM_UNIQUE_ID_BYTES: u32 = 128;
+pub const WFPT_TILE_LIST_CAP: u32 = 16;
+pub const WFPT_TILE_NO_LIST: u32 = 0xffffffff;
 
 pub const WFPT_OK: c_int = 0;
 pub const WFPT_ERR_INVALID_ARGUMENT: c_int = -1;
@@ -70,6 +72,7 @@
 pub const WFPT_FLAG_ENV_NEE: u32 = 1 << 16;
 pub const WFPT_FLAG_MIS: u32 = 1 << 17;
 pub const WFPT_FLAG_ENV_MIS: u32 = 1 << 18;
+pub const WFPT_FLAG_NO_TILE_LISTS: u32 = 1 << 19;
 
 #[repr(C)]
 #[derive(Copy, Clone, Debug, Default)]
@@ -329,5 +332,9 @@
     pub fn wfpt_debug_read_stamps(ctx: *mut wfpt_ctx, out: *mut u64, reset: c_int) -> c_int;
     pub fn wfpt_debug_read_stamps_ex(ctx: *mut wfpt_ctx, which: c_int, out: *mut u64, reset: c_int) -> c_int;
     pub fn wfpt_debug_bvh4(nodes: *const wfpt_bvh_node, n_nodes: u32, counts: *mut u32) -> c_int;
+    pub fn wfpt_tile_lists_host(nodes_ch: *const f32, n_nodes: u32, camera: *const wfpt_gpu_camera, inv_proj: *const f32, view: *const f32, width: u32, height: u32, tile_rank: u32, tile_world: u32, records: *mut u32, n_tiles: u32) -> c_int;
+    pub fn wfpt_debug_nodes_ch(nodes: *const wfpt_bvh_node, n_nodes: u32, camera: *const wfpt_gpu_camera, nodes_ch: *mut f32) -> c_int;
+    pub fn wfpt_debug_read_tile_lists(ctx: *mut wfpt_ctx, records: *mut u32, n_tiles: *mut u32) -> c_int;
+    pub fn wfpt_tile_lists_timing_ms(ctx: *mut wfpt_ctx, ms_last: *mut f32, builds: *mut u32) -> c_int;
     pub fn wfpt_build_info() -> *const c_char;
 }
```

Result: faster. 24280, median of 6 (+3.2%).
